# Grid2op/grid2op

Hardware: AMD Instinct MI355X
Metric: env steps/sec (batched DoNothing) (higher is better)
Workload: dtype f64; 1 GPU; l2rpn_case14_sandbox AC Newton-Raphson DoNothing env.step, batch=4096 lanes per GPU; env=l2rpn_case14_sandbox, lanes_per_gpu=4096, total_lanes=4096, env_steps_per_launch=16, observations=every env step -> HBM, cascade=False, kernels=grid-specialised at run time (gpf_jit_enable), parallelism=static lane shards x1, no collective

## Files before the change

grid2op_amd/aot/85d4f0b0125d.h:

```cpp
#define GPF_JIT_SET_G(v) do { (v).n_sub = 118; (v).n_busbar = 2; (v).nb_tot = 236; (v).n_line = 186; (v).n_gen = 62; (v).n_load = 99; (v).n_sto = 7; (v).n_shunt = 14; (v).dim_topo = 540; (v).n_inj = 364; (v).n_out = 2574; (v).n_chron = 322; (v).sn_mva = 0x1p+0; (v).inv_sn_mva = 0x1p+0; } while (0)
#define GPF_JIT_SET_OO(v) do { (v).p_or = 0; (v).q_or = 186; (v).v_or = 372; (v).a_or = 558; (v).th_or = 744; (v).p_ex = 930; (v).q_ex = 1116; (v).v_ex = 1302; (v).a_ex = 1488; (v).th_ex = 1674; (v).gen_p = 1860; (v).gen_q = 1922; (v).gen_v = 1984; (v).gen_th = 2046; (v).load_p = 2108; (v).load_q = 2207; (v).load_v = 2306; (v).load_th = 2405; (v).sto_p = 2504; (v).sto_q = 2511; (v).sto_v = 2518; (v).sto_th = 2525; (v).sh_p = 2532; (v).sh_q = 2546; (v).sh_v = 2560; (v).inj_gen_p = 0; (v).inj_gen_vm = 62; (v).inj_load_p = 124; (v).inj_load_q = 223; (v).inj_sto_p = 322; (v).inj_sto_q = 329; (v).inj_sh_p = 336; (v).inj_sh_q = 350; } while (0)
#define GPF_JIT_SET_SYM(v) do { (v).n = 118; (v).nslot = 674; (v).nslot_y = 476; (v).n_levels = 13; (v).back_off = 2628; (v).n_prog = 3188; (v).scale_off = 2361; (v).n_scale = 267; (v).nslot_lu = 652; (v).n_up = 179; (v).rslot0 = 674; (v).back_first = 11; (v).static_connected = 1; (v).fl[0].n_fwd = 74; (v).fl[0].n_scale = 0; (v).fl[0].n_scale_rhs = 0; (v).fl[0].n_back = 17; (v).fl[0].scale_off = 2400; (v).fl[0].back_off = 2400; (v).fl[0].rhs_field0 = 10784; (v).fl[0].n_words = 3008; (v).fl[0].wave_closed = 1; (v).fl[0].solo_fwd = 0; (v).fl[0].solo_back = 0; (v).fl[1].n_fwd = 39; (v).fl[1].n_scale = 0; (v).fl[1].n_scale_rhs = 0; (v).fl[1].n_back = 11; (v).fl[1].scale_off = 2560; (v).fl[1].back_off = 2560; (v).fl[1].rhs_field0 = 10784; (v).fl[1].n_words = 3392; (v).fl[1].wave_closed = 1; (v).fl[1].solo_fwd = 0; (v).fl[1].solo_back = 0; (v).fl[2].n_fwd = 22; (v).fl[2].n_scale = 0; (v).fl[2].n_scale_rhs = 0; (v).fl[2].n_back = 6; (v).fl[2].scale_off = 2944; (v).fl[2].back_off = 2944; (v).fl[2].rhs_field0 = 10784; (v).fl[2].n_words = 3840; (v).fl[2].wave_closed = 1; (v).fl[2].solo_fwd = 0; (v).fl[2].solo_back = 0; (v).fl[3].n_fwd = 13; (v).fl[3].n_scale = 0; (v).fl[3].n_scale_rhs = 0; (v).fl[3].n_back = 6; (v).fl[3].scale_off = 3584; (v).fl[3].back_off = 3584; (v).fl[3].rhs_field0 = 10784; (v).fl[3].n_words = 5632; (v).fl[3].wave_closed = 1; (v).fl[3].solo_fwd = 7680; (v).fl[3].solo_back = 63; } while (0)
#define GPF_JIT_SET_SO(v) do { (v).n_dbl = 2982; (v).n_int = 6548; (v).n_int_hot = 4024; (v).br_y = 0; (v).br_bdc = 1488; (v).sub_vn_kv = 1674; (v).shunt_fact = 1792; (v).gen_min_q = 1806; (v).gen_max_q = 1868; (v).line_vn = 1930; (v).load_vn = 2674; (v).gen_vn = 2774; (v).sto_vn = 2836; (v).shunt_vn = 2844; (v).line_ka = 2302; (v).gen_qmin_tot = 2858; (v).gen_qmax_tot = 2920; (v).gen_cnt = 5944; (v).dc_inv = -1; (v).line_or_pos = 4024; (v).line_ex_pos = 4212; (v).line_or_sub = 4400; (v).line_ex_sub = 4588; (v).br_slot = 4776; (v).gen_pos = 5520; (v).gen_sub = 5584; (v).gen_slack = 5648; (v).load_pos = 5712; (v).load_sub = 5812; (v).sto_pos = 5912; (v).sto_sub = 5920; (v).shunt_sub = 5928; (v).pair_rc = 3188; (v).up = 3664; (v).prog = 0; (v).pos_line = 6008; } while (0)
```

grid2op_amd/aot/c7e3abcd557d.h:

```cpp
#define GPF_JIT_SET_G(v) do { (v).n_sub = 36; (v).n_busbar = 2; (v).nb_tot = 72; (v).n_line = 59; (v).n_gen = 22; (v).n_load = 37; (v).n_sto = 0; (v).n_shunt = 6; (v).dim_topo = 177; (v).n_inj = 130; (v).n_out = 844; (v).n_chron = 118; (v).sn_mva = 0x1p+0; (v).inv_sn_mva = 0x1p+0; } while (0)
#define GPF_JIT_SET_OO(v) do { (v).p_or = 0; (v).q_or = 59; (v).v_or = 118; (v).a_or = 177; (v).th_or = 236; (v).p_ex = 295; (v).q_ex = 354; (v).v_ex = 413; (v).a_ex = 472; (v).th_ex = 531; (v).gen_p = 590; (v).gen_q = 612; (v).gen_v = 634; (v).gen_th = 656; (v).load_p = 678; (v).load_q = 715; (v).load_v = 752; (v).load_th = 789; (v).sto_p = 826; (v).sto_q = 826; (v).sto_v = 826; (v).sto_th = 826; (v).sh_p = 826; (v).sh_q = 832; (v).sh_v = 838; (v).inj_gen_p = 0; (v).inj_gen_vm = 22; (v).inj_load_p = 44; (v).inj_load_q = 81; (v).inj_sto_p = 118; (v).inj_sto_q = 118; (v).inj_sh_p = 118; (v).inj_sh_q = 124; } while (0)
#define GPF_JIT_SET_SYM(v) do { (v).n = 36; (v).nslot = 196; (v).nslot_y = 146; (v).n_levels = 8; (v).back_off = 752; (v).n_prog = 920; (v).scale_off = 676; (v).n_scale = 76; (v).nslot_lu = 188; (v).n_up = 55; (v).rslot0 = 196; (v).back_first = 6; (v).static_connected = 1; (v).fl[0].n_fwd = 23; (v).fl[0].n_scale = 0; (v).fl[0].n_scale_rhs = 0; (v).fl[0].n_back = 6; (v).fl[0].scale_off = 768; (v).fl[0].back_off = 768; (v).fl[0].rhs_field0 = 3136; (v).fl[0].n_words = 1024; (v).fl[0].wave_closed = 1; (v).fl[0].solo_fwd = 0; (v).fl[0].solo_back = 0; (v).fl[1].n_fwd = 13; (v).fl[1].n_scale = 0; (v).fl[1].n_scale_rhs = 0; (v).fl[1].n_back = 3; (v).fl[1].scale_off = 896; (v).fl[1].back_off = 896; (v).fl[1].rhs_field0 = 3136; (v).fl[1].n_words = 1216; (v).fl[1].wave_closed = 1; (v).fl[1].solo_fwd = 0; (v).fl[1].solo_back = 0; (v).fl[2].n_fwd = 8; (v).fl[2].n_scale = 0; (v).fl[2].n_scale_rhs = 0; (v).fl[2].n_back = 3; (v).fl[2].scale_off = 1152; (v).fl[2].back_off = 1152; (v).fl[2].rhs_field0 = 3136; (v).fl[2].n_words = 1664; (v).fl[2].wave_closed = 1; (v).fl[2].solo_fwd = 0; (v).fl[2].solo_back = 0; (v).fl[3].n_fwd = 8; (v).fl[3].n_scale = 0; (v).fl[3].n_scale_rhs = 0; (v).fl[3].n_back = 3; (v).fl[3].scale_off = 2304; (v).fl[3].back_off = 2304; (v).fl[3].rhs_field0 = 3136; (v).fl[3].n_words = 3584; (v).fl[3].wave_closed = 1; (v).fl[3].solo_fwd = 255; (v).fl[3].solo_back = 7; } while (0)
#define GPF_JIT_SET_SO(v) do { (v).n_dbl = 964; (v).n_int = 2020; (v).n_int_hot = 1180; (v).br_y = 0; (v).br_bdc = 472; (v).sub_vn_kv = 532; (v).shunt_fact = 568; (v).gen_min_q = 574; (v).gen_max_q = 596; (v).line_vn = 618; (v).load_vn = 854; (v).gen_vn = 892; (v).sto_vn = 914; (v).shunt_vn = 914; (v).line_ka = 736; (v).gen_qmin_tot = 920; (v).gen_qmax_tot = 942; (v).gen_cnt = 1816; (v).dc_inv = -2; (v).line_or_pos = 1180; (v).line_ex_pos = 1240; (v).line_or_sub = 1300; (v).line_ex_sub = 1360; (v).br_slot = 1420; (v).gen_pos = 1656; (v).gen_sub = 1680; (v).gen_slack = 1704; (v).load_pos = 1728; (v).load_sub = 1768; (v).sto_pos = 1808; (v).sto_sub = 1808; (v).shunt_sub = 1808; (v).pair_rc = 920; (v).up = 1068; (v).prog = 0; (v).pos_line = 1840; } while (0)
```

grid2op_amd/aot/f41e44a3ff50.h:

```cpp
#define GPF_JIT_SET_G(v) do { (v).n_sub = 118; (v).n_busbar = 2; (v).nb_tot = 236; (v).n_line = 186; (v).n_gen = 62; (v).n_load = 91; (v).n_sto = 7; (v).n_shunt = 14; (v).dim_topo = 532; (v).n_inj = 348; (v).n_out = 2542; (v).n_chron = 306; (v).sn_mva = 0x1p+0; (v).inv_sn_mva = 0x1p+0; } while (0)
#define GPF_JIT_SET_OO(v) do { (v).p_or = 0; (v).q_or = 186; (v).v_or = 372; (v).a_or = 558; (v).th_or = 744; (v).p_ex = 930; (v).q_ex = 1116; (v).v_ex = 1302; (v).a_ex = 1488; (v).th_ex = 1674; (v).gen_p = 1860; (v).gen_q = 1922; (v).gen_v = 1984; (v).gen_th = 2046; (v).load_p = 2108; (v).load_q = 2199; (v).load_v = 2290; (v).load_th = 2381; (v).sto_p = 2472; (v).sto_q = 2479; (v).sto_v = 2486; (v).sto_th = 2493; (v).sh_p = 2500; (v).sh_q = 2514; (v).sh_v = 2528; (v).inj_gen_p = 0; (v).inj_gen_vm = 62; (v).inj_load_p = 124; (v).inj_load_q = 215; (v).inj_sto_p = 306; (v).inj_sto_q = 313; (v).inj_sh_p = 320; (v).inj_sh_q = 334; } while (0)
#define GPF_JIT_SET_SYM(v) do { (v).n = 118; (v).nslot = 674; (v).nslot_y = 476; (v).n_levels = 13; (v).back_off = 2628; (v).n_prog = 3188; (v).scale_off = 2361; (v).n_scale = 267; (v).nslot_lu = 652; (v).n_up = 179; (v).rslot0 = 674; (v).back_first = 11; (v).static_connected = 1; (v).fl[0].n_fwd = 74; (v).fl[0].n_scale = 0; (v).fl[0].n_scale_rhs = 0; (v).fl[0].n_back = 17; (v).fl[0].scale_off = 2400; (v).fl[0].back_off = 2400; (v).fl[0].rhs_field0 = 10784; (v).fl[0].n_words = 3008; (v).fl[0].wave_closed = 1; (v).fl[0].solo_fwd = 0; (v).fl[0].solo_back = 0; (v).fl[1].n_fwd = 39; (v).fl[1].n_scale = 0; (v).fl[1].n_scale_rhs = 0; (v).fl[1].n_back = 11; (v).fl[1].scale_off = 2560; (v).fl[1].back_off = 2560; (v).fl[1].rhs_field0 = 10784; (v).fl[1].n_words = 3392; (v).fl[1].wave_closed = 1; (v).fl[1].solo_fwd = 0; (v).fl[1].solo_back = 0; (v).fl[2].n_fwd = 22; (v).fl[2].n_scale = 0; (v).fl[2].n_scale_rhs = 0; (v).fl[2].n_back = 6; (v).fl[2].scale_off = 2944; (v).fl[2].back_off = 2944; (v).fl[2].rhs_field0 = 10784; (v).fl[2].n_words = 3840; (v).fl[2].wave_closed = 1; (v).fl[2].solo_fwd = 0; (v).fl[2].solo_back = 0; (v).fl[3].n_fwd = 13; (v).fl[3].n_scale = 0; (v).fl[3].n_scale_rhs = 0; (v).fl[3].n_back = 6; (v).fl[3].scale_off = 3584; (v).fl[3].back_off = 3584; (v).fl[3].rhs_field0 = 10784; (v).fl[3].n_words = 5632; (v).fl[3].wave_closed = 1; (v).fl[3].solo_fwd = 7680; (v).fl[3].solo_back = 63; } while (0)
#define GPF_JIT_SET_SO(v) do { (v).n_dbl = 2974; (v).n_int = 6524; (v).n_int_hot = 4024; (v).br_y = 0; (v).br_bdc = 1488; (v).sub_vn_kv = 1674; (v).shunt_fact = 1792; (v).gen_min_q = 1806; (v).gen_max_q = 1868; (v).line_vn = 1930; (v).load_vn = 2674; (v).gen_vn = 2766; (v).sto_vn = 2828; (v).shunt_vn = 2836; (v).line_ka = 2302; (v).gen_qmin_tot = 2850; (v).gen_qmax_tot = 2912; (v).gen_cnt = 5928; (v).dc_inv = -1; (v).line_or_pos = 4024; (v).line_ex_pos = 4212; (v).line_or_sub = 4400; (v).line_ex_sub = 4588; (v).br_slot = 4776; (v).gen_pos = 5520; (v).gen_sub = 5584; (v).gen_slack = 5648; (v).load_pos = 5712; (v).load_sub = 5804; (v).sto_pos = 5896; (v).sto_sub = 5904; (v).shunt_sub = 5912; (v).pair_rc = 3188; (v).up = 3664; (v).prog = 0; (v).pos_line = 5992; } while (0)
```

grid2op_amd/aot/f5e9fdf573e3.h:

```cpp
#define GPF_JIT_SET_G(v) do { (v).n_sub = 14; (v).n_busbar = 2; (v).nb_tot = 28; (v).n_line = 20; (v).n_gen = 6; (v).n_load = 11; (v).n_sto = 0; (v).n_shunt = 1; (v).dim_topo = 57; (v).n_inj = 36; (v).n_out = 271; (v).n_chron = 34; (v).sn_mva = 0x1.9p+6; (v).inv_sn_mva = 0x1.47ae147ae147bp-7; } while (0)
#define GPF_JIT_SET_OO(v) do { (v).p_or = 0; (v).q_or = 20; (v).v_or = 40; (v).a_or = 60; (v).th_or = 80; (v).p_ex = 100; (v).q_ex = 120; (v).v_ex = 140; (v).a_ex = 160; (v).th_ex = 180; (v).gen_p = 200; (v).gen_q = 206; (v).gen_v = 212; (v).gen_th = 218; (v).load_p = 224; (v).load_q = 235; (v).load_v = 246; (v).load_th = 257; (v).sto_p = 268; (v).sto_q = 268; (v).sto_v = 268; (v).sto_th = 268; (v).sh_p = 268; (v).sh_q = 269; (v).sh_v = 270; (v).inj_gen_p = 0; (v).inj_gen_vm = 6; (v).inj_load_p = 12; (v).inj_load_q = 23; (v).inj_sto_p = 34; (v).inj_sto_q = 34; (v).inj_sh_p = 34; (v).inj_sh_q = 35; } while (0)
#define GPF_JIT_SET_SYM(v) do { (v).n = 14; (v).nslot = 66; (v).nslot_y = 54; (v).n_levels = 5; (v).back_off = 242; (v).n_prog = 300; (v).scale_off = 218; (v).n_scale = 24; (v).nslot_lu = 62; (v).n_up = 20; (v).rslot0 = 66; (v).back_first = 3; (v).static_connected = 1; (v).fl[0].n_fwd = 8; (v).fl[0].n_scale = 0; (v).fl[0].n_scale_rhs = 0; (v).fl[0].n_back = 1; (v).fl[0].scale_off = 288; (v).fl[0].back_off = 288; (v).fl[0].rhs_field0 = 1056; (v).fl[0].n_words = 384; (v).fl[0].wave_closed = 1; (v).fl[0].solo_fwd = 0; (v).fl[0].solo_back = 0; (v).fl[1].n_fwd = 5; (v).fl[1].n_scale = 0; (v).fl[1].n_scale_rhs = 0; (v).fl[1].n_back = 1; (v).fl[1].scale_off = 384; (v).fl[1].back_off = 384; (v).fl[1].rhs_field0 = 1056; (v).fl[1].n_words = 576; (v).fl[1].wave_closed = 1; (v).fl[1].solo_fwd = 0; (v).fl[1].solo_back = 0; (v).fl[2].n_fwd = 5; (v).fl[2].n_scale = 0; (v).fl[2].n_scale_rhs = 0; (v).fl[2].n_back = 1; (v).fl[2].scale_off = 768; (v).fl[2].back_off = 768; (v).fl[2].rhs_field0 = 1056; (v).fl[2].n_words = 1024; (v).fl[2].wave_closed = 1; (v).fl[2].solo_fwd = 0; (v).fl[2].solo_back = 0; (v).fl[3].n_fwd = 5; (v).fl[3].n_scale = 0; (v).fl[3].n_scale_rhs = 0; (v).fl[3].n_back = 1; (v).fl[3].scale_off = 1536; (v).fl[3].back_off = 1536; (v).fl[3].rhs_field0 = 1056; (v).fl[3].n_words = 2304; (v).fl[3].wave_closed = 1; (v).fl[3].solo_fwd = 31; (v).fl[3].solo_back = 1; } while (0)
#define GPF_JIT_SET_SO(v) do { (v).n_dbl = 516; (v).n_int = 676; (v).n_int_hot = 396; (v).br_y = 0; (v).br_bdc = 160; (v).sub_vn_kv = 180; (v).shunt_fact = 194; (v).gen_min_q = 196; (v).gen_max_q = 202; (v).line_vn = 208; (v).load_vn = 288; (v).gen_vn = 300; (v).sto_vn = 306; (v).shunt_vn = 306; (v).line_ka = 248; (v).gen_qmin_tot = 308; (v).gen_qmax_tot = 314; (v).gen_cnt = 608; (v).dc_inv = 320; (v).line_or_pos = 396; (v).line_ex_pos = 416; (v).line_or_sub = 436; (v).line_ex_sub = 456; (v).br_slot = 476; (v).gen_pos = 556; (v).gen_sub = 564; (v).gen_slack = 572; (v).load_pos = 580; (v).load_sub = 592; (v).sto_pos = 604; (v).sto_sub = 604; (v).shunt_sub = 604; (v).pair_rc = 300; (v).up = 356; (v).prog = 0; (v).pos_line = 616; } while (0)
```

grid2op_amd/csrc/gridpf_capi.hip:

```cpp
#include <hip/hip_runtime.h>

#include <algorithm>
#include <chrono>
#include <cmath>
#include <cstdio>
#include <cstdlib>
#include <cstring>
#include <climits>
#include <map>
#include <mutex>
#include <string>
#include <vector>

#include "gridpf_engine.hpp"
#include "gridpf_redispatch.hpp"
#include "gridpf_topo.hpp"
#include "gridpf_topo_mask.hpp"

namespace gpf {
__global__ void fanout_kernel(GridDev g, Bufs b, int src, int dst0, int n_dst, const int* __restrict__ out_lines) {
  const int k = blockIdx.x;
  if (k >= n_dst) return;
  const int dst = dst0 + k;
  const int tid = threadIdx.x;
// ... 90 lines not shown
}

namespace {

template <typename T>
hipError_t rows_to_host(const gpf_engine* e, T* host, const DevArr<T>& arr, size_t stride, int lane0, int n) {
  if (!host || stride == 0) return hipSuccess;
  return hipMemcpyAsync(host, arr.p + (size_t)lane0 * stride, (size_t)n * stride * sizeof(T), hipMemcpyDeviceToHost, e->stream);
}
template <typename T>
hipError_t rows_to_device(const gpf_engine* e, const DevArr<T>& arr, const T* host, size_t stride, int lane0, int n) {
  if (!host || stride == 0) return hipSuccess;
  return hipMemcpyAsync(arr.p + (size_t)lane0 * stride, host, (size_t)n * stride * sizeof(T), hipMemcpyHostToDevice, e->stream);
}
template <typename T>
hipError_t rows_copy(const gpf_engine* e, const DevArr<T>& arr, size_t stride, int src, int dst, int n) {
  if (stride == 0) return hipSuccess;
  return hipMemcpyAsync(arr.p + (size_t)dst * stride, arr.p + (size_t)src * stride, (size_t)n * stride * sizeof(T), hipMemcpyDeviceToDevice, e->stream);
}

void topo_unmoved(gpf_engine* e, int lane0, int n) {
  if (e->ta_n_moved == 0) return;
  for (int k = lane0; k < lane0 + n; ++k) if (e->ta_moved[k]) { e->ta_moved[k] = 0; --e->ta_n_moved; }
}

gpf::TopoDev topo_dev(const gpf_engine* e) {
  const gpf::GridDev& g = e->g;
  gpf::TopoDev d{};
  d.dim_topo = g.dim_topo; d.n_line = g.n_line; d.n_sub = g.n_sub; d.n_shunt = g.n_shunt; d.n_busbar = g.n_busbar;
  d.line_or_pos = g.line_or_pos; d.line_ex_pos = g.line_ex_pos; d.shunt_sub = g.shunt_sub;
  d.topo = e->topo.p; d.shunt_bus = e->shunt_bus.p; d.cooldown = e->cooldown.p; d.topo0 = e->topo0.p; d.episode = e->episode.p; d.done = e->done.p;
  return d;
}

gpf::TopoLanes topo_lanes(const gpf_engine* e) {
  gpf::TopoLanes t{};
  t.act = e->ta_act.p; t.sub_cd = e->ta_sub_cd.p; t.last_bus = e->ta_last_bus.p; t.flags = e->ta_flags.p; t.aff = e->ta_aff.p;
  t.ep_snap = e->ta_ep_snap.p; t.list = e->ta_list.p; t.list_rows = e->ta_list_rows.p; t.pos_sub = e->ta_pos_sub.p; t.pos_other = e->ta_pos_other.p;
  t.n_slot = e->ta_n_slot;
  return t;
}

void count_lane(const gpf_engine* e, const int* topo, const int* shunt_bus, int& nb, int& nj, int& mb) {
  const gpf::GridDev& g = e->g;
  std::vector<unsigned char> act(g.nb_tot, 0), type(g.nb_tot, 0);
  auto mark = [&](int sub, int local) -> int {
    if (local < 1 || local > g.n_busbar) return -1;
    int gb = sub + (local - 1) * g.n_sub;
    act[gb] = 1;
    return gb;
  };
  for (int l = 0; l < g.n_line; ++l) {
    int bo = topo[e->h_line_or_pos[l]], be = topo[e->h_line_ex_pos[l]];
    if (bo >= 1 && be >= 1) { mark(e->h_line_or_sub[l], bo); mark(e->h_line_ex_sub[l], be); }
  }
  for (int i = 0; i < g.n_gen; ++i) {
    int gb = mark(e->h_gen_sub[i], topo[e->h_gen_pos[i]]);
    if (gb >= 0) type[gb] = std::max<unsigned char>(type[gb], e->h_gen_slack[i] ? 2 : 1);
  }
  for (int i = 0; i < g.n_load; ++i) mark(e->h_load_sub[i], topo[e->h_load_pos[i]]);
  for (int i = 0; i < g.n_sto; ++i) mark(e->h_sto_sub[i], topo[e->h_sto_pos[i]]);
  if (shunt_bus)
    for (int i = 0; i < g.n_shunt; ++i) mark(e->h_shunt_sub[i], shunt_bus[i]);
  nb = 0;
  nj = 0;
  for (int b = 0; b < g.nb_tot; ++b) {
    if (!act[b]) continue;
    ++nb;
    if (type[b] == 0) nj += 2;
    else if (type[b] == 1) nj += 1;
  }
  mb = 1;
  for (int s = 0; s < g.n_sub; ++s) {
    int c = 0;
    for (int k = 0; k < g.n_busbar; ++k) c += act[s + k * g.n_sub];
    mb = std::max(mb, c);
  }
}



bool upload_flats(const gpf::Symbolic& S, DevArr<int>& buf, gpf::SymDev& D, int lane_opt = 0) {
  D.rslot0 = S.rslot0;
  for (int k = 0; k < 4; ++k) { D.flat[k] = nullptr; D.fl[k] = gpf::FlatDev{}; }
  if (!gpf::flat_fits(S)) return true;
  std::vector<int> all;
  size_t off[4];
  for (int k = 0; k < 4; ++k) {
    static std::mutex cache_mu;
    static std::unordered_map<std::string, gpf::FlatProg> cache;
    std::string key;
    if (lane_opt > 0) {
      key = std::to_string(S.slot_row.size()) + ":" + std::to_string(S.slot_col.size()) + ":" + std::to_string(S.prog.size()) + ":";
      key.append(reinterpret_cast<const char*>(S.slot_row.data()), S.slot_row.size() * sizeof(int));
      key.append(reinterpret_cast<const char*>(S.slot_col.data()), S.slot_col.size() * sizeof(int));
      key.append(reinterpret_cast<const char*>(S.prog.data()), S.prog.size() * sizeof(int));
      key += "/" + std::to_string(16 << k) + "/" + std::to_string(lane_opt) + "/" + std::to_string(S.gj_lv0) + "/" + std::to_string(S.nslot_lu);
    }
    gpf::FlatProg F;
    bool have = false;
    if (lane_opt > 0) {
      std::lock_guard<std::mutex> lk(cache_mu);
      auto hit = cache.find(key);
      if (hit != cache.end()) { F = hit->second; have = true; }
    }
    if (!have) {
      F = gpf::build_flat(S, 16 << k, lane_opt);
      if (lane_opt > 0) {
        std::lock_guard<std::mutex> lk(cache_mu);
        if (cache.size() < 64) cache.emplace(key, F);
      }
    }
    off[k] = all.size();
    all.insert(all.end(), F.words.begin(), F.words.end());
    gpf::FlatDev& f = D.fl[k];
    f.n_fwd = F.n_fwd; f.n_scale = F.n_scale; f.n_scale_rhs = F.n_scale_rhs; f.n_back = F.n_back; f.scale_off = F.scale_off;
    f.back_off = F.back_off; f.rhs_field0 = F.rhs_field0; f.n_words = (int)F.words.size(); f.wave_closed = F.wave_closed ? 1 : 0;
    f.solo_fwd = (int)F.solo_fwd; f.solo_back = (int)F.solo_back;
  }
  if (buf.upload(all.data(), all.size()) != hipSuccess) return false;
  for (int k = 0; k < 4; ++k) D.flat[k] = buf.p + off[k];
  if (g_dry_create) {
    static int dry_words;
    for (int k = 0; k < 4; ++k) D.flat[k] = &dry_words;
  }
  return true;
}

gpf::Symbolic build_symbolic_resident(const gpf::GridDev& g, int n_rows, int n_line, const int* lo, const int* le, bool yb_in_lds);

int topo_class_of(gpf_engine* e, const int* topo, const int* shunt_bus) {
  const gpf::GridDev& g = e->g;
  if (e->no_classes || g.n_busbar < 2 || e->classes.size() >= 8192) return -1;
  const int nbb = g.n_busbar;
  std::string key((size_t)2 * g.n_line + (size_t)g.n_sub * nbb, '\0');
  auto bb = [&](int v) { return v >= 2 && v <= nbb ? v : 1; };
  for (int l = 0; l < g.n_line; ++l) {
    key[2 * l] = (char)bb(topo[e->h_line_or_pos[l]]);
    key[2 * l + 1] = (char)bb(topo[e->h_line_ex_pos[l]]);
  }
  char* used = &key[(size_t)2 * g.n_line];
  auto mark = [&](int sub, int v) { if (v >= 1 && v <= nbb) used[(size_t)sub * nbb + (v - 1)] = 1; };
  for (int l = 0; l < g.n_line; ++l) { mark(e->h_line_or_sub[l], key[2 * l]); mark(e->h_line_ex_sub[l], key[2 * l + 1]); }
  for (int i = 0; i < g.n_gen; ++i) mark(e->h_gen_sub[i], topo[e->h_gen_pos[i]]);
  for (int i = 0; i < g.n_load; ++i) mark(e->h_load_sub[i], topo[e->h_load_pos[i]]);
  for (int i = 0; i < g.n_sto; ++i) mark(e->h_sto_sub[i], topo[e->h_sto_pos[i]]);
  if (shunt_bus) for (int i = 0; i < g.n_shunt; ++i) mark(e->h_shunt_sub[i], shunt_bus[i]);
  std::string elem(used, (size_t)g.n_sub * nbb);
  for (int s_ = 0; s_ < g.n_sub; ++s_) used[(size_t)s_ * nbb] = 1;
  auto it = e->class_of_key.find(key);
  if (it != e->class_of_key.end()) return it->second;
  std::vector<int> node_of((size_t)g.n_sub * nbb, -1);
  int n_nodes = g.n_sub;
  for (int s_ = 0; s_ < g.n_sub; ++s_) node_of[(size_t)s_ * nbb] = s_;
  for (int s_ = 0; s_ < g.n_sub; ++s_)
    for (int k = 1; k < nbb; ++k) if (used[(size_t)s_ * nbb + k]) node_of[(size_t)s_ * nbb + k] = n_nodes++;
  if (n_nodes > 32767) return -1;
  std::vector<int> lo(g.n_line), le(g.n_line);
  for (int l = 0; l < g.n_line; ++l) {
    lo[l] = node_of[(size_t)e->h_line_or_sub[l] * nbb + (key[2 * l] - 1)];
    le[l] = node_of[(size_t)e->h_line_ex_sub[l] * nbb + (key[2 * l + 1] - 1)];
  }
  gpf::Symbolic S = build_symbolic_resident(g, n_nodes, g.n_line, lo.data(), le.data(), true);
  if (S.nslot > 65535 || !gpf::flat_fits(S)) return -1;
  auto c = std::make_unique<gpf_engine::TopoClassHost>();
  std::vector<int> fi;
  auto puti = [&fi](const int* v, size_t n) { int off = (int)fi.size(); fi.insert(fi.end(), v, v + n); while (fi.size() & 3) fi.push_back(0); return off; };
  const int o_prog = puti(S.prog.data(), S.prog.size());
  std::vector<int> rc(S.nslot_y);
  for (int k = 0; k < S.nslot_y; ++k) rc[k] = S.slot_row[k] | (S.slot_col[k] << 16);
  const int o_rc = puti(rc.data(), rc.size());
  const std::vector<int> upv = gpf::build_upairs(S);
  const int o_up = puti(upv.data(), upv.size());
  const int o_br = puti(S.br_slot.data(), S.br_slot.size());
  const int o_no = puti(node_of.data(), node_of.size());
  if (c->tables.upload(fi.data(), fi.size()) != hipSuccess) return -1;
  c->n_nodes = n_nodes; c->nslot = S.nslot; c->nslot_y = S.nslot_y;
  gpf::SymDev& D = c->dev.sym;
  D = e->sym_dev;
  D.n = S.n; D.nslot = S.nslot; D.nslot_lu = S.nslot_lu; D.nslot_y = S.nslot_y; D.n_levels = S.n_levels; D.back_off = S.back_off; D.back_first = S.back_first;
  D.scale_off = S.scale_off; D.n_scale = S.n_scale; D.n_prog = (int)S.prog.size();
  {
    std::vector<int> comp(n_nodes);
    for (int i = 0; i < n_nodes; ++i) comp[i] = i;
    auto find = [&](int x) { while (comp[x] != x) { comp[x] = comp[comp[x]]; x = comp[x]; } return x; };
    for (int l = 0; l < g.n_line; ++l) comp[find(lo[l])] = find(le[l]);
    int root = -1;
    bool one = true;
    for (int s_ = 0; s_ < g.n_sub && one; ++s_)
      for (int k = 0; k < nbb && one; ++k)
        if (elem[(size_t)s_ * nbb + k]) {
          const int r = find(node_of[(size_t)s_ * nbb + k]);
          if (root < 0) root = r; else one = (r == root);
        }
    D.static_connected = one ? 1 : 0;
  }
  D.prog = c->tables.p + o_prog;
  if (!upload_flats(S, c->flat, D) || !D.fl[3].wave_closed) return -1;
  c->dev.pair_rc = c->tables.p + o_rc; c->dev.up = c->tables.p + o_up; c->dev.br_slot = c->tables.p + o_br; c->dev.node_of = c->tables.p + o_no;
  D.n_up = (int)upv.size() / 2;
  const int id = (int)e->classes.size();
// ... 2321 lines not shown
```

grid2op_amd/csrc/gridpf_sparse.hpp:

```cpp
#pragma once
#include <type_traits>
#include "gridpf_common.hpp"

namespace gpf {

struct StatOff {
  int n_dbl, n_int;
  int n_int_hot;
  int br_y, br_bdc, sub_vn_kv, shunt_fact, gen_min_q, gen_max_q;
  int line_vn, load_vn, gen_vn, sto_vn, shunt_vn;
  int line_ka;
  int gen_qmin_tot, gen_qmax_tot;
  int gen_cnt;
  int dc_inv;
  int line_or_pos, line_ex_pos, line_or_sub, line_ex_sub, br_slot, gen_pos, gen_sub, gen_slack, load_pos, load_sub, sto_pos,
      sto_sub, shunt_sub, pair_rc, up, prog;
  int pos_line;
};
#define GPF_STATOFF_INTS(X) X(n_dbl) X(n_int) X(n_int_hot) X(br_y) X(br_bdc) X(sub_vn_kv) X(shunt_fact) X(gen_min_q) X(gen_max_q) X(line_vn) X(load_vn) \
  X(gen_vn) X(sto_vn) X(shunt_vn) X(line_ka) X(gen_qmin_tot) X(gen_qmax_tot) X(gen_cnt) X(dc_inv) X(line_or_pos) X(line_ex_pos) X(line_or_sub) \
  X(line_ex_sub) X(br_slot) X(gen_pos) X(gen_sub) X(gen_slack) X(load_pos) X(load_sub) X(sto_pos) X(sto_sub) X(shunt_sub) X(pair_rc) X(up) X(prog) X(pos_line)
static_assert(sizeof(StatOff) == sizeof(int) * (0 GPF_STATOFF_INTS(GPF_COUNT_FIELD)), "GPF_STATOFF_INTS must list every field of StatOff");
template <class T, bool IN_LDS>
struct SP {
  const T* p;
  __device__ __forceinline__ T operator[](int i) const { return IN_LDS ? p[i] : (T)gptr(p)[i]; }
  __device__ __forceinline__ double4 ld4(size_t off) const {
    if (IN_LDS) return *reinterpret_cast<const double4*>(p + off);
    typedef double v4d_ __attribute__((ext_vector_type(4)));
    const v4d_ v = *(GPF_GLOBAL const v4d_*)(gptr(p) + off);
    return make_double4(v.x, v.y, v.z, v.w);
  }
};
template <int STAGE>
struct StatView {
  static constexpr bool ALL = STAGE == 2, HOT = STAGE >= 1;
  SP<double, ALL> br_y, br_bdc, sub_vn_kv, shunt_fact, gen_min_q, gen_max_q, line_vn, line_ka, load_vn, gen_vn, sto_vn, shunt_vn, dc_inv, gen_qmin_tot, gen_qmax_tot;
  SP<int, ALL> line_or_pos, line_ex_pos, line_or_sub, line_ex_sub, br_slot, gen_pos, gen_sub, gen_slack, load_pos, load_sub,
      sto_pos, sto_sub, shunt_sub, gen_cnt, pos_line;
  SP<int, HOT> pair_rc;
  SP<int, HOT> up;
  SP<int, HOT> prog;
  SP<int, false> node_of;
  SP<double, false> dc_inv_g;
};
template <int STAGE>
__device__ inline void stat_view(StatView<STAGE>& v, const StatOff& o, const double* d, const int* i) {
  v.br_y.p = d + o.br_y; v.br_bdc.p = d + o.br_bdc; v.sub_vn_kv.p = d + o.sub_vn_kv; v.shunt_fact.p = d + o.shunt_fact;
  v.gen_min_q.p = d + o.gen_min_q; v.gen_max_q.p = d + o.gen_max_q;
  v.dc_inv.p = d + (o.dc_inv >= 0 ? o.dc_inv : 0);
  v.gen_qmin_tot.p = d + o.gen_qmin_tot; v.gen_qmax_tot.p = d + o.gen_qmax_tot; v.gen_cnt.p = i + o.gen_cnt;
  v.line_vn.p = d + o.line_vn; v.line_ka.p = d + o.line_ka; v.load_vn.p = d + o.load_vn; v.gen_vn.p = d + o.gen_vn; v.sto_vn.p = d + o.sto_vn; v.shunt_vn.p = d + o.shunt_vn;
  v.line_or_pos.p = i + o.line_or_pos; v.line_ex_pos.p = i + o.line_ex_pos; v.line_or_sub.p = i + o.line_or_sub;
  v.line_ex_sub.p = i + o.line_ex_sub; v.br_slot.p = i + o.br_slot; v.gen_pos.p = i + o.gen_pos; v.gen_sub.p = i + o.gen_sub;
  v.gen_slack.p = i + o.gen_slack; v.load_pos.p = i + o.load_pos; v.load_sub.p = i + o.load_sub; v.sto_pos.p = i + o.sto_pos;
  v.sto_sub.p = i + o.sto_sub; v.shunt_sub.p = i + o.shunt_sub; v.pos_line.p = i + o.pos_line; v.pair_rc.p = i + o.pair_rc; v.up.p = i + o.up; v.prog.p = i + o.prog;
  v.node_of.p = nullptr;
}
__host__ __device__ inline size_t stat_bytes(const StatOff& o, int tier, bool nb1, int n_flat) {
  if (tier == 0) return 0;
  if (!nb1) return ((size_t)o.n_int_hot * 4 + 15) & ~(size_t)15;
  const size_t ints = (size_t)((tier == 2 ? o.n_int : o.n_int_hot) - o.pair_rc) + (size_t)n_flat;
  return ((tier == 2 ? (size_t)o.n_dbl * 8 : 0) + ints * 4 + 15) & ~(size_t)15;
}

struct FlatDev {
  int n_fwd, n_scale, n_scale_rhs, n_back, scale_off, back_off, rhs_field0, n_words;
  int wave_closed;
  int solo_fwd, solo_back;
};
#define GPF_FLATDEV_INTS(X) X(n_fwd) X(n_scale) X(n_scale_rhs) X(n_back) X(scale_off) X(back_off) X(rhs_field0) X(n_words) X(wave_closed) X(solo_fwd) X(solo_back)
static_assert(sizeof(FlatDev) == sizeof(int) * (0 GPF_FLATDEV_INTS(GPF_COUNT_FIELD)), "GPF_FLATDEV_INTS must list every field of FlatDev");
__host__ __device__ constexpr int gw_index(int gw) { return gw >= 128 ? 3 : gw >= 64 ? 2 : gw >= 32 ? 1 : 0; }

struct SymDev {
  int n, nslot, nslot_y, n_levels, back_off, n_prog, scale_off, n_scale;
  int nslot_lu;
  int n_up;
  int rslot0;
  const int* flat[4];
  FlatDev fl[4];
  int back_first;
  int static_connected;
  const int* prog;
  const double* dc_inv_g;
  const double* stat_dbl;
  const int* stat_int;
  StatOff so;
};

#define GPF_SYMDEV_INTS(X) X(n) X(nslot) X(nslot_y) X(n_levels) X(back_off) X(n_prog) X(scale_off) X(n_scale) X(nslot_lu) X(n_up) X(rslot0) X(back_first) \
  X(static_connected)

struct TopoClassDev {
  SymDev sym;
  const int* pair_rc;
  const int* up;
  const int* br_slot;
  const int* node_of;
};

struct DevParamsS {
  GridDev g;
  Bufs b;
  OutOff oo;
  SymDev sym;
  const TopoClassDev* classes;
  int tc_rows;
  int tc_nslot, tc_nslot_y;
  int dcf;
  EnvDyn env;
};

#ifdef GPF_TIMING
constexpr int GPF_NSTAMP = 40;
constexpr int GPF_NPASS_T = 48;
constexpr int GPF_WORK_ROW = GPF_NSTAMP + GPF_NPASS_T;
static __shared__ long long gpf_pass_t[GPF_NPASS_T];
struct Stamps { long long v[GPF_NSTAMP]; };
#define GPF_STAMPS(k) do { stamps.v[(k)] = (long long)__builtin_readcyclecounter(); } while (0)
#define GPF_STAMPS_PARAM , Stamps& stamps
#define GPF_STAMPS_ARG , stamps
#define GPF_STAMPS_DECL Stamps stamps; for (int k_ = 0; k_ < GPF_NSTAMP; ++k_) stamps.v[k_] = 0; \
  for (int k_ = threadIdx.x; k_ < GPF_NPASS_T; k_ += blockDim.x) gpf_pass_t[k_] = 0
#define GPF_STAMPS_FLUSH(inst_) do { if (tid == 0) { for (int k_ = 0; k_ < GPF_NSTAMP; ++k_) P->b.work[(size_t)(inst_) * GPF_WORK_ROW + k_] = (double)stamps.v[k_]; \
    for (int k_ = 0; k_ < GPF_NPASS_T; ++k_) P->b.work[(size_t)(inst_) * GPF_WORK_ROW + GPF_NSTAMP + k_] = (double)gpf_pass_t[k_]; } } while (0)
#else
#define GPF_STAMPS(k) do {} while (0)
#define GPF_STAMPS_PARAM
#define GPF_STAMPS_ARG
#define GPF_STAMPS_DECL do {} while (0)
#define GPF_STAMPS_FLUSH(inst_) do {} while (0)
#endif

#ifndef GPF_WAVE_SYNC
#define GPF_SYNC() __syncthreads()
#else
#define GPF_SYNC() do { __builtin_amdgcn_fence(__ATOMIC_RELEASE, "wavefront"); __builtin_amdgcn_wave_barrier(); \
                        __builtin_amdgcn_fence(__ATOMIC_ACQUIRE, "wavefront"); } while (0)
#endif

#ifndef GPF_HARD_SYNC
#define GPF_PF2_ON true
#define GPF_LSYNC() do { if (GW > WAVE) asm volatile("s_waitcnt lgkmcnt(0)\n\ts_barrier" ::: "memory"); else { asm volatile("" ::: "memory"); __builtin_amdgcn_wave_barrier(); asm volatile("" ::: "memory"); } } while (0)
#else
#define GPF_PF2_ON false
#define GPF_LSYNC() GPF_SYNC()
#endif

#define GPF_SYNC_IF(cond) do { if (GW > WAVE || (cond)) GPF_SYNC(); else GPF_LSYNC(); } while (0)

typedef short i16;

#ifndef GPF_JIT
__device__ __forceinline__ void pin_sgpr(int& x) { x = __builtin_amdgcn_readfirstlane(x); asm volatile("" : "+s"(x)); }
#define GPF_SPEC_G(v) do {} while (0)
#define GPF_SPEC_OO(v) do {} while (0)
#define GPF_SPEC_SYM(v) do {} while (0)
#define GPF_SPEC_SO(v) do {} while (0)
#else
__device__ __forceinline__ void pin_sgpr(int&) {}
#define GPF_SPEC_G(v) GPF_JIT_SET_G(v)
#define GPF_SPEC_OO(v) GPF_JIT_SET_OO(v)
#define GPF_SPEC_SYM(v) GPF_JIT_SET_SYM(v)
#define GPF_SPEC_SO(v) GPF_JIT_SET_SO(v)
#endif

template <int NB>
struct CarveP {
  static constexpr int BS = 2 * NB;
  double* A;
  double* Yb;
  double* rhs;
  double *vm, *va, *e, *f, *Psp, *Qsp;
  double* ivm;
  double *Sre, *Sim;
  double* Gs;
  double* inj;
  double* Adc;
  int* btype;
  int* vidx;
  int* lab;
  int* topo;
  i16 *lor_b, *lex_b, *gen_b, *load_b, *sto_b, *sh_b;
  i8* sub_bb;
  float* out_l;
};

template <int NB>
__host__ __device__ inline size_t lds_bytes_instance(const GridDev& g, int nslot, int nslot_y, bool stage_inj, int n_rows = -1, bool dcf = false) {
  constexpr int BS = 2 * NB;
  const size_t rows = n_rows > 0 ? (size_t)n_rows : (size_t)g.n_sub;
  const size_t nbus = rows * NB;
  const size_t rs0 = (size_t)nslot > (3 * rows + 1) / 2 ? (size_t)nslot : (3 * rows + 1) / 2;
  size_t a_d = NB == 1 ? (rs0 + rows) * 4 : (size_t)nslot * BS * BS;
  const size_t topo_d = (((size_t)g.dim_topo + 1) / 2 + 2) & ~(size_t)1;
  if (a_d < topo_d) a_d = topo_d;
  const size_t nd = a_d + (size_t)nslot_y * NB * NB * 2 + (NB == 1 ? 7 * nbus : rows * BS + 8 * nbus) + (stage_inj ? (size_t)g.n_inj : 0) +
// ... 333 lines not shown
#pragma unroll
        for (int m = 0; m < BS; ++m) acc = fma(Di[m], bp[m], acc);
      }
      GPF_LSYNC();
      if (on) rhs[(size_t)p * BS + (it % BS)] = acc;
      GPF_LSYNC();
    }
    }
    for (int it = tid; it < n_c * B2; it += GW) {
      const int o = it / B2, r = (it % B2) / BS, q = it % BS;
      const unsigned w0 = (unsigned)prog[c_off + 2 * o];
      const int u = prog[c_off + 2 * o + 1] & 0xffff;
      const double* Al = A + (size_t)(w0 >> 16) * B2 + r * BS;
      const double* Au = A + (size_t)u * B2 + q;
      double acc = 0.0;
#pragma unroll
      for (int m = 0; m < BS; ++m) acc = fma(Al[m], Au[m * BS], acc);
      atomicAdd(&A[(size_t)(w0 & 0xffffu) * B2 + r * BS + q], -acc);
    }
    for (int it = tid; it < n_r * BS; it += GW) {
      const int o = it / BS, r = it % BS;
      const unsigned w0 = (unsigned)prog[r_off + 2 * o];
      const int p = prog[r_off + 2 * o + 1];
      const double* Al = A + (size_t)(w0 & 0xffffu) * B2 + r * BS;
      const double* bp = rhs + (size_t)p * BS;
      double acc = 0.0;
#pragma unroll
      for (int m = 0; m < BS; ++m) acc = fma(Al[m], bp[m], acc);
      atomicAdd(&rhs[(size_t)(w0 >> 16) * BS + r], -acc);
    }
    GPF_LSYNC();
  }
#ifdef GPF_TIMING
  const long long t_lu1 = __builtin_readcyclecounter();
#endif
  for (int lv = S.n_levels - 1; lv >= 0; --lv) {
    const int ent_off = prog[S.back_off + 2 * lv], n_ent = prog[S.back_off + 2 * lv + 1];
    for (int it = tid; it < n_ent * BS; it += GW) {
      const unsigned w = (unsigned)prog[ent_off + 2 * (it / BS)];
      const int p = prog[ent_off + 2 * (it / BS) + 1], r = it % BS;
      const double* Au = A + (size_t)(w & 0xffffu) * B2 + r * BS;
      const double* xj = rhs + (size_t)(w >> 16) * BS;
      double acc = 0.0;
#pragma unroll
      for (int m = 0; m < BS; ++m) acc = fma(Au[m], xj[m], acc);
      atomicAdd(&rhs[(size_t)p * BS + r], -acc);
    }
    GPF_LSYNC();
  }
#ifdef GPF_TIMING
  if (dbg) { dbg[0] = t_lu1 - t_lu0; dbg[1] = (long long)__builtin_readcyclecounter() - t_lu1; }
#endif
  return ok;
}

constexpr int GPF_WR_CAP_F = 6, GPF_WR_CAP_B = 2;
template <bool ON> struct FlatWords { };
template <> struct FlatWords<true> { unsigned f[2 * GPF_WR_CAP_F], b[2 * GPF_WR_CAP_B]; };
#ifdef GPF_NO_WORDS_RES
template <int NB, int IPW, int WPI> constexpr bool flat_words_ct() { return false; }
#else
template <int NB, int IPW, int WPI> constexpr bool flat_words_ct() { return NB == 1 && IPW > 1 && WPI == 1; }
#endif
__device__ __forceinline__ bool flat_words_fit(const FlatDev& F) { return F.n_fwd <= GPF_WR_CAP_F && F.n_back <= GPF_WR_CAP_B; }
template <int GW, class PP>
__device__ __forceinline__ void flat_words_load(FlatWords<false>&, const FlatDev&, PP, int) {}
template <int GW, class PP>
__device__ __forceinline__ void flat_words_load(FlatWords<true>& W, const FlatDev& F, PP prog, int tid) {
  const bool fit = flat_words_fit(F);
#pragma unroll
  for (int k = 0; k < GPF_WR_CAP_F; ++k) {
    const bool on_f = fit && k < F.n_fwd;
    W.f[2 * k] = on_f ? (unsigned)prog[2 * tid + 2 * GW * k] : 0xffffffffu;
    W.f[2 * k + 1] = on_f ? (unsigned)prog[2 * tid + 2 * GW * k + 1] : 0u;
  }
#pragma unroll
  for (int k = 0; k < GPF_WR_CAP_B; ++k) {
    const bool on_b = fit && k < F.n_back;
    W.b[2 * k] = on_b ? (unsigned)prog[F.back_off + 2 * tid + 2 * GW * k] : 0xffffffffu;
    W.b[2 * k + 1] = on_b ? (unsigned)prog[F.back_off + 2 * tid + 2 * GW * k + 1] : 0u;
  }
}

template <int GW, class PP = const int*, bool RES = false>
__device__ inline bool block_lu_flat(const FlatDev& F, PP prog, double* __restrict__ A, size_t HS, int tid, long long* dbg = nullptr,
                                     const FlatWords<RES>* W = nullptr) {
#ifdef GPF_TIMING
  const long long t_lu0 = __builtin_readcyclecounter();
#endif
  bool ok = true;
#ifdef GPF_PF2_IG
  constexpr bool PF2 = GPF_PF2_ON && (GW > WAVE || (GW <= 32 && !std::is_same<PP, const int*>::value));
#else
  constexpr bool PF2 = GPF_PF2_ON && GW > WAVE;
#endif
  char* const a0 = reinterpret_cast<char*>(A);
  char* const a1 = a0 + HS * 8;
#define FL_LD2(base, f) (*reinterpret_cast<const double2*>((base) + (f)))
#define FL_D(base, f) (reinterpret_cast<double*>((base) + (f)))
#ifdef GPF_TIMING
#define GPF_PASS_T(i_) do { if (dbg && tid == 0 && (i_) < GPF_NPASS_T) gpf_pass_t[(i_)] = (long long)__builtin_readcyclecounter(); } while (0)
#else
#define GPF_PASS_T(i_) do {} while (0)
#endif
  GPF_PASS_T(0);
  auto fwd_item = [&](const unsigned w0, const unsigned w1) {
    if (w0 != 0xffffffffu) {
      const unsigned fd = w0 & 0xffffu, fl = w0 >> 16, fu = w1 & 0xffffu, fp = w1 >> 16;
      const double2 dA = FL_LD2(a0, fp), dB = FL_LD2(a1, fp), lA = FL_LD2(a0, fl), lB = FL_LD2(a1, fl);
      const double2 uA = FL_LD2(a0, fu), uB = FL_LD2(a1, fu);
      const double rd = -fast_rcp(fma(dA.x, dB.y, -dA.y * dB.x));
      const double t00 = fma(lA.x, dB.y, -lA.y * dB.x), t01 = fma(lA.y, dA.x, -lA.x * dA.y);
      const double t10 = fma(lB.x, dB.y, -lB.y * dB.x), t11 = fma(lB.y, dA.x, -lB.x * dA.y);
      double* d0_ = FL_D(a0, fd);
      double* d1_ = FL_D(a1, fd);
      atomicAdd(&d0_[0], fma(t00, uA.x, t01 * uB.x) * rd);
      atomicAdd(&d1_[0], fma(t10, uA.x, t11 * uB.x) * rd);
      if (fd < (unsigned)F.rhs_field0) {
        atomicAdd(&d0_[1], fma(t00, uA.y, t01 * uB.y) * rd);
        atomicAdd(&d1_[1], fma(t10, uA.y, t11 * uB.y) * rd);
      }
    }
  };
#define GPF_WALK(n_, at0_, MASK_, NEXT_SOLO_, ITEM_, TB_, WR_, CAP_)                                                                                 \
  {                                                                                                                                \
    const unsigned solo_ = GW > WAVE ? (unsigned)(MASK_) : 0u;                                                                     \
    const int n_pass_ = (n_);                                                                                                      \
    auto step_ = [&](const unsigned a_, const unsigned b_, const int k) {                                                          \
      const bool so_ = GW > WAVE && k < 32 && ((solo_ >> (k & 31)) & 1u);                                                          \
      if (!so_ || tid < WAVE) ITEM_(a_, b_);                                                                                       \
      const bool sn_ = so_ && (k + 1 < n_pass_ ? (k + 1 < 32 && ((solo_ >> ((k + 1) & 31)) & 1u)) : (GW > WAVE && (NEXT_SOLO_)));  \
      if (sn_) { asm volatile("" ::: "memory"); __builtin_amdgcn_wave_barrier(); asm volatile("" ::: "memory"); }                 \
      else GPF_LSYNC();                                                                                                            \
      GPF_PASS_T((TB_) + k);                                                                                                       \
    };                                                                                                                             \
    if constexpr (RES) {                                   \
      _Pragma("unroll")                                                                                                            \
      for (int k = 0; k < (CAP_); ++k)                                                                                             \
        if (k < n_pass_) step_(W->WR_[2 * k], W->WR_[2 * k + 1], k);                                                               \
    } else {                                                                                                                       \
    int at = (at0_) + 2 * tid;                                                                                                     \
    unsigned p0 = (unsigned)prog[at], p1 = (unsigned)prog[at + 1];                                                                 \
    if (PF2) {                                                                                                                     \
      at += 2 * GW;                                                                                                                \
      unsigned q0 = (unsigned)prog[at], q1 = (unsigned)prog[at + 1], r0, r1;                                                       \
      for (int k = 0; k < n_pass_; k += 3) {                                                                                       \
        at += 2 * GW; r0 = (unsigned)prog[at]; r1 = (unsigned)prog[at + 1];                                                        \
        step_(p0, p1, k);                                                                                                          \
        if (k + 1 >= n_pass_) break;                                                                                               \
        at += 2 * GW; p0 = (unsigned)prog[at]; p1 = (unsigned)prog[at + 1];                                                        \
        step_(q0, q1, k + 1);                                                                                                      \
        if (k + 2 >= n_pass_) break;                                                                                               \
        at += 2 * GW; q0 = (unsigned)prog[at]; q1 = (unsigned)prog[at + 1];                                                        \
        step_(r0, r1, k + 2);                                                                                                      \
      }                                                                                                                            \
    } else {                                                                                                                       \
      for (int k = 0; k < n_pass_; ++k) {                                                                                          \
        at += 2 * GW;                                                                                                              \
        const unsigned n0 = (unsigned)prog[at], n1 = (unsigned)prog[at + 1];                           \
        step_(p0, p1, k);                                                                                                          \
        p0 = n0; p1 = n1;                                                                                                          \
      }                                                                                                                            \
    }                                                                                                                              \
    }                                                                                                                              \
  }
  GPF_WALK(F.n_fwd, 0, F.solo_fwd, F.n_back > 0 && (F.solo_back & 1), fwd_item, 1, f, GPF_WR_CAP_F)
#ifdef GPF_TIMING
  const long long t_lu1 = __builtin_readcyclecounter();
#endif
  auto back_item = [&](const unsigned w0, const unsigned w1) {
    if (w0 != 0xffffffffu) {
      const unsigned fu = w0 & 0xffffu, fj = w0 >> 16, fdj = fj - (unsigned)F.rhs_field0;
      const double2 uA = FL_LD2(a0, fu), uB = FL_LD2(a1, fu), dA = FL_LD2(a0, fdj), dB = FL_LD2(a1, fdj);
      const double s0 = *FL_D(a0, fj), s1 = *FL_D(a1, fj);
      const double rd = fast_rcp(fma(dA.x, dB.y, -dA.y * dB.x));
      const double x0 = fma(dB.y, s0, -dA.y * s1) * rd, x1 = fma(dA.x, s1, -dB.x * s0) * rd;
      atomicAdd(FL_D(a0, w1), -fma(uA.x, x0, uA.y * x1));
      atomicAdd(FL_D(a1, w1), -fma(uB.x, x0, uB.y * x1));
    }
  };
  GPF_WALK(F.n_back, F.back_off, F.solo_back, false, back_item, 1 + F.n_fwd, b, GPF_WR_CAP_B)
#ifdef GPF_TIMING
  if (dbg) { dbg[0] = t_lu1 - t_lu0; dbg[1] = (long long)__builtin_readcyclecounter() - t_lu1; }
#endif
  return ok;
}

template <int GW, bool FACTOR, bool COMPACT, class PP = const int*, bool RES = false>
__device__ inline bool scalar_lu_flat(const FlatDev& F, PP prog, double* __restrict__ A, double* __restrict__ fac, int tid,
                                      long long* dbg = nullptr, const FlatWords<RES>* W = nullptr) {
#ifdef GPF_TIMING
  const long long t_lu0 = __builtin_readcyclecounter();
#endif
  bool ok = true;
#ifdef GPF_PF2_IG
  constexpr bool PF2 = GPF_PF2_ON && (GW > WAVE || (GW <= 32 && !std::is_same<PP, const int*>::value));
#else
  constexpr bool PF2 = GPF_PF2_ON && GW > WAVE;
#endif
  char* const a0 = reinterpret_cast<char*>(A);
  char* const fb = reinterpret_cast<char*>(fac);
  auto facp = [&](unsigned f) -> double* { return reinterpret_cast<double*>(fb + (COMPACT ? (f >> 1) : f)); };
  auto fwd_item = [&](const unsigned w0, const unsigned w1) {
    const unsigned fd = w0 & 0xffffu, fl = w0 >> 16, fu = w1 & 0xffffu, fp = w1 >> 16;
    const bool is_r = (int)fd >= F.rhs_field0;
    if (w0 != 0xffffffffu && (FACTOR || is_r)) {
      const double d = *facp(fp), al = *facp(fl);
      const double x = is_r ? *FL_D(a0, fu) : *facp(fu);
      double* dst = is_r ? FL_D(a0, fd) : facp(fd);
      atomicAdd(dst, -(al * x) * fast_rcp(d));
    }
  };
#undef GPF_PASS_T
#define GPF_PASS_T(i_) do {} while (0)
  GPF_WALK(F.n_fwd, 0, F.solo_fwd, F.n_back > 0 && (F.solo_back & 1), fwd_item, 0, f, GPF_WR_CAP_F)
#ifdef GPF_TIMING
  const long long t_lu1 = __builtin_readcyclecounter();
#endif
  auto back_item = [&](const unsigned w0, const unsigned w1) {
    if (w0 != 0xffffffffu) {
      const unsigned fj = w0 >> 16;
      atomicAdd(FL_D(a0, w1), -(*facp(w0 & 0xffffu) * *FL_D(a0, fj)) * fast_rcp(*facp(fj - (unsigned)F.rhs_field0)));
    }
  };
  GPF_WALK(F.n_back, F.back_off, F.solo_back, false, back_item, 0, b, GPF_WR_CAP_B)
#ifdef GPF_TIMING
  if (dbg) { dbg[0] = t_lu1 - t_lu0; dbg[1] = (long long)__builtin_readcyclecounter() - t_lu1; }
#endif
  return ok;
}
#undef GPF_PASS_T
#undef GPF_WALK
#undef FL_LD2
#undef FL_D

struct SolveCtl {
  bool inj_staged;
  bool topo_staged;
  bool reuse;
  bool dcf;
  bool write_bus;
  bool sums_done;
  bool warm;
  bool otraj;
  int orow;
  bool write_topo;
  bool inj_regs;
  float r_lp0, r_lq0, r_lp1, r_lq1, r_pp, r_vm;
  bool tc_rebuild;
};
struct TopoState {
  int status;
  int nb;
  bool dc_base;
  int dc_out;
  bool gen_base;
  int tc[2];
};

constexpr int YR_PASSES = 4;
template <int NB, int STAGE, int IPW, int WPI, bool TC, bool YR = false>
__device__ inline int solve_instance_sparse(const DevParamsS* __restrict__ P, const SymDev& S, const FlatDev& FL, const StatView<STAGE>& sv, CarveP<NB>& c, double2* yreg, unsigned* rcreg,
                                            const FlatWords<flat_words_ct<NB, IPW, WPI>()>& FW, int inst, int is_dc, int max_iter,
                                            double tol_pu, int tid, const SolveCtl& ctl, TopoState& ts, int& n_iter_out, int& nb_out, float& a_or_first GPF_STAMPS_PARAM) {
  typedef Grp<IPW, WPI> G;
  constexpr int GW = G::GW;
  constexpr int BS = 2 * NB;
  constexpr int B2 = BS * BS;
  GridDev g_loc = P->g;
  GPF_SPEC_G(g_loc);
  pin_sgpr(g_loc.n_sub); pin_sgpr(g_loc.n_line); pin_sgpr(g_loc.n_gen); pin_sgpr(g_loc.n_load); pin_sgpr(g_loc.n_sto);
  pin_sgpr(g_loc.n_shunt); pin_sgpr(g_loc.dim_topo); pin_sgpr(g_loc.nb_tot);
  const GridDev& g = g_loc;
  const Bufs& b = P->b;
#ifdef GPF_JIT
  OutOff oo_loc = P->oo;
  GPF_SPEC_OO(oo_loc);
  const OutOff& oo = oo_loc;
#else
  const OutOff& oo = P->oo;
#endif
  const int nsub = g.n_sub;
  const int nbus = TC ? S.n : nsub * NB;
  constexpr int GWA = WPI > 1 ? WAVE : GW;
  const bool acc_lane = WPI == 1 || tid < WAVE;
  const bool wave1 = WPI > 1 && tid >= WAVE;
  const size_t HS = ((size_t)S.rslot0 + S.n) * 2;
  auto bel = [&](int slot, int r, int col) -> double* {
    return BS == 2 ? c.A + (size_t)r * HS + (size_t)slot * 2 + col : c.A + (size_t)slot * B2 + r * BS + col;
  };
  auto rhsT = [&](int i) -> double* { return BS == 2 ? c.A + ((size_t)S.rslot0 + i) * 2 : c.rhs + (size_t)(i / NB) * BS + 2 * (i % NB); };
  auto rhsV = [&](int i) -> double* { return BS == 2 ? c.A + HS + ((size_t)S.rslot0 + i) * 2 : c.rhs + (size_t)(i / NB) * BS + 2 * (i % NB) + 1; };
  auto SreP = [&](int i) -> double* { return BS == 2 ? c.A + ((size_t)S.rslot0 + i) * 2 + 1 : c.Sre + i; };
  auto SimP = [&](int i) -> double* { return BS == 2 ? c.A + HS + ((size_t)S.rslot0 + i) * 2 + 1 : c.Sim + i; };
  auto EF = [&](int i) -> double2 { return NB == 1 ? reinterpret_cast<const double2*>(c.e)[i] : make_double2(c.e[i], c.f[i]); };
  auto setEF = [&](int i, double e_, double f_) { if (NB == 1) reinterpret_cast<double2*>(c.e)[i] = make_double2(e_, f_); else { c.e[i] = e_; c.f[i] = f_; } };
  const auto topo_g = gptr(b.topo) + (size_t)inst * g.dim_topo;
  const auto shb = gptr(b.shunt_bus) + (size_t)inst * g.n_shunt;
  n_iter_out = 0;
  nb_out = 0;
  c.out_l = nullptr;
  GPF_STAMPS(0);
  const auto inj_g = gptr(b.inj) + (size_t)inst * g.n_inj;
  if (STAGE && !ctl.inj_staged) {
    for (int i = tid; i < g.n_inj; i += GW) c.inj[i] = inj_g[i];
  }
  const bool reuse = ctl.reuse;
  const bool dc_kept = reuse && ctl.dcf && NB == 1;
  const bool warm = reuse && ctl.warm && !is_dc;
#ifdef GPF_NO_NWR
  constexpr bool NWR = false;
#else
  constexpr bool NWR = NB == 1 && WPI == 1 && !YR;
#endif
  const bool nwr = NWR && !is_dc && nbus <= GW && S.n_up <= GW;
  const bool fast_pre = nwr && reuse && ctl.sums_done && !warm && !TC && S.so.dc_inv != -1 && G::block_all_u(ts.dc_base && ts.dc_out < 0);
#define GPF_INJ(i_) (STAGE ? c.inj[(i_)] : (double)inj_g[(i_)])
// ... 194 lines not shown
  if (!dc_skip) for (int i = tid; i < (NB == 1 ? S.nslot : S.nslot_lu) * B2; i += GW) c.A[i] = 0.0;
  if (do_y) for (int i = tid; i < S.nslot_y * NB * NB * 2; i += GW) ydst[i] = 0.0;
  GPF_LSYNC();
  if (acc_lane)
  for (int l = tid; l < g.n_line; l += GWA) {
    const int f = c.lor_b[l], t = c.lex_b[l];
    if (f < 0) continue;
    const int bi = lidx(f), bj = lidx(t);
    const int sff = sv.br_slot[4 * l + 0], sft = sv.br_slot[4 * l + 1], stf = sv.br_slot[4 * l + 2], stt = sv.br_slot[4 * l + 3];
    if (do_y) {
      const double4 ya = sv.br_y.ld4((size_t)8 * l), yb = sv.br_y.ld4((size_t)8 * l + 4);
      double* y;
      y = ydst + ((size_t)sff * NB * NB + bi * NB + bi) * 2; atomicAdd(&y[0], ya.x); atomicAdd(&y[1], ya.y);
      y = ydst + ((size_t)sft * NB * NB + bi * NB + bj) * 2; atomicAdd(&y[0], ya.z); atomicAdd(&y[1], ya.w);
      y = ydst + ((size_t)stf * NB * NB + bj * NB + bi) * 2; atomicAdd(&y[0], yb.x); atomicAdd(&y[1], yb.y);
      y = ydst + ((size_t)stt * NB * NB + bj * NB + bj) * 2; atomicAdd(&y[0], yb.z); atomicAdd(&y[1], yb.w);
    }
    if (f != t && !dc_skip) {
      const double bb = sv.br_bdc[l];
      const bool ff_ = c.btype[f] != BT_REF, tf_ = c.btype[t] != BT_REF;
      const int rf = 2 * bi, rt = 2 * bj;
      if (ff_) atomicAdd(bel(sff, rf, rf), bb);
      if (tf_) atomicAdd(bel(stt, rt, rt), bb);
      if (ff_ && tf_) {
        atomicAdd(bel(sft, rf, rt), -bb);
        atomicAdd(bel(stf, rt, rf), -bb);
      }
    }
  }
  if (do_y && acc_lane) {
    for (int s = tid; s < g.n_shunt; s += GWA) {
      const int bu = c.sh_b[s];
      if (bu >= 0) {
        const int bi = lidx(bu);
        const int sub = (NB == 1) ? bu : bu / NB;
        const double fct = sv.shunt_fact[s] * inv_sn;
        double* y = ydst + ((size_t)sub * NB * NB + bi * NB + bi) * 2;
        atomicAdd(&y[0], GPF_INJ(oo.inj_sh_p + s) * fct);
        atomicAdd(&y[1], -GPF_INJ(oo.inj_sh_q + s) * fct);
      }
    }
  }
  GPF_LSYNC();
  if (YR && do_y) {
#pragma unroll
    for (int k = 0; k < YR_PASSES; ++k) {
      const int pr = tid + k * GW;
      const unsigned w0 = pr < S.n_up ? (unsigned)sv.up[2 * pr] : 0u, w1 = pr < S.n_up ? (unsigned)sv.up[2 * pr + 1] : 0u;
      rcreg[2 * k] = w0; rcreg[2 * k + 1] = w1;
      yreg[2 * k] = pr < S.n_up ? *reinterpret_cast<const double2*>(ydst + (size_t)(w1 & 0xffffu) * 2) : make_double2(0.0, 0.0);
      yreg[2 * k + 1] = pr < S.n_up ? *reinterpret_cast<const double2*>(ydst + (size_t)(w1 >> 16) * 2) : make_double2(0.0, 0.0);
    }
    yreg[2 * YR_PASSES] = tid < nbus ? *reinterpret_cast<const double2*>(ydst + (size_t)tid * 2) : make_double2(0.0, 0.0);
    GPF_LSYNC();
  }
  }
  if (!fuse_dc)
  for (int i = tid; i < nbus; i += GW) {
    const int sub = (NB == 1) ? i : i / NB, bi = lidx(i);
    const int bt = c.btype[i];
    const bool th_live = (bt == BT_PQ || bt == BT_PV);
    if (!dc_skip) {
      if (!th_live) *bel(sub, 2 * bi, 2 * bi) = 1.0;
      *bel(sub, 2 * bi + 1, 2 * bi + 1) = 1.0;
    }
    *rhsT(i) = th_live ? (c.Psp[i] - c.Gs[i]) : 0.0;
    *rhsV(i) = 0.0;
  }
  if (!fuse_dc) GPF_LSYNC();
  }
  GPF_STAMPS(3);
  const int* const flat_g = STAGE == 0 ? sv.prog.p : S.flat[gw_index(GW)];
  constexpr bool PROG_LDS = STAGE >= 1 && IPW == 1;
  constexpr bool WRES = flat_words_ct<NB, IPW, WPI>();
  const bool wres = WRES && flat_words_fit(FL);
  auto lu_ac = [&](long long* dbg) -> bool {
    if (BS == 2) {
      if (WRES && wres) return block_lu_flat<GW, decltype(gptr(flat_g)), WRES>(FL, gptr(flat_g), c.A, HS, tid, dbg, &FW);
      if (PROG_LDS) return block_lu_flat<GW>(FL, sv.prog.p, c.A, HS, tid, dbg);
      return block_lu_flat<GW>(FL, gptr(flat_g), c.A, HS, tid, dbg);
    }
    if (STAGE >= 1) return block_lu_solve<BS, GW>(S, sv.prog.p, c.A, c.rhs, tid, dbg);
    return block_lu_solve<BS, GW>(S, gptr(sv.prog.p), c.A, c.rhs, tid, dbg);
  };
  auto lu_dc = [&](long long* dbg) -> bool {
    if (dc_kept) {
      if (WRES && wres) return scalar_lu_flat<GW, false, true, decltype(gptr(flat_g)), WRES>(FL, gptr(flat_g), c.A, c.Adc, tid, dbg, &FW);
      if (PROG_LDS) return scalar_lu_flat<GW, false, true>(FL, sv.prog.p, c.A, c.Adc, tid, dbg);
      return scalar_lu_flat<GW, false, true>(FL, gptr(flat_g), c.A, c.Adc, tid, dbg);
    }
    if (WRES && wres) return scalar_lu_flat<GW, true, false, decltype(gptr(flat_g)), WRES>(FL, gptr(flat_g), c.A, c.A, tid, dbg, &FW);
    if (PROG_LDS) return scalar_lu_flat<GW, true, false>(FL, sv.prog.p, c.A, c.A, tid, dbg);
    return scalar_lu_flat<GW, true, false>(FL, gptr(flat_g), c.A, c.A, tid, dbg);
  };
  if (!warm && !fuse_dc) {
#ifdef GPF_TIMING
    bool ok = dc_inv ? true : (NB == 1) ? lu_dc(&stamps.v[20])
                                        : lu_ac(&stamps.v[20]);
#else
    bool ok = dc_inv ? true : (NB == 1) ? lu_dc(nullptr) : lu_ac(nullptr);
#endif
    for (int i = tid; i < nbus; i += GW) {
      double th;
      if (dc_inv) {
        auto row_times_rhs = [&](const auto tab) -> double {
          double t0 = 0.0, t1 = 0.0;
          for (int k0 = 0; k0 < nbus; k0 += MVC) {
            double a_[MVC], r_[MVC];
#pragma unroll
            for (int q = 0; q < MVC; ++q) {
              const int k = k0 + q < nbus ? k0 + q : nbus - 1;
              a_[q] = tab[k * nbus + i];
              r_[q] = *rhsT(k);
            }
#pragma unroll
            for (int q = 0; q < MVC; q += 2) {
              if (k0 + q < nbus) t0 = fma(a_[q], r_[q], t0);
              if (k0 + q + 1 < nbus) t1 = fma(a_[q + 1], r_[q + 1], t1);
            }
          }
          return t0 + t1;
        };
        th = S.so.dc_inv >= 0 ? row_times_rhs(sv.dc_inv) : row_times_rhs(sv.dc_inv_g);
      } else if (NB == 1) {
        const double d = dc_kept ? c.Adc[i] : c.A[(size_t)i * 2];
        if (!(fabs(d) > 1e-300) || !(fabs(d) < 1e300)) ok = false;
        th = *rhsT(i) * fast_rcp(d);
      } else th = *rhsT(i);
      const int bt = c.btype[i];
      c.va[i] = (bt == BT_PQ || bt == BT_PV) ? th : 0.0;
      if (bt != BT_OFF && !(fabs(th) < 1e300)) ok = false;
    }
    if (NB == 1 && ctl.dcf && !dc_skip)
      for (int q = tid; q < S.nslot; q += GW) c.Adc[q] = c.A[(size_t)q * 2];
    GPF_LSYNC();
    if (WPI == 1 && dc_inv && G::block_any_u(ts.dc_out >= 0)) {
      const int lo_ = ts.dc_out >= 0 ? ts.dc_out : 0;
      const int f_ = sv.line_or_sub[lo_], t_ = sv.line_ex_sub[lo_];
      const double bl = ts.dc_out >= 0 ? sv.br_bdc[lo_] : 0.0;
      const bool f_ref = c.btype[f_] == BT_REF, t_ref = c.btype[t_] == BT_REF;
      const double dth = c.va[f_] - c.va[t_];
      const double xff = f_ref ? 0.0 : dcinv(f_ * nbus + f_), xtt = t_ref ? 0.0 : dcinv(t_ * nbus + t_);
      const double xft = (f_ref || t_ref) ? 0.0 : dcinv(t_ * nbus + f_);
      const double den = 1.0 - bl * (xff - 2.0 * xft + xtt);
      if (!(fabs(den) > 1e-12)) ok = false;
      const double kk = bl * dth / den;
      for (int i = tid; i < nbus; i += GW) {
        const int bt = c.btype[i];
        const double u_ = (f_ref ? 0.0 : dcinv(f_ * nbus + i)) - (t_ref ? 0.0 : dcinv(t_ * nbus + i));
        if (bt == BT_PQ || bt == BT_PV) c.va[i] += u_ * kk;
      }
      GPF_LSYNC();
    }
    if (status == 0 && G::any(!ok)) status = 4;
    if (G::block_all_u(status != 0)) return status;
  }
  GPF_STAMPS(4);

  int it = 0;
  if (!is_dc) {
    bool converged = false;
    bool done = status != 0;
    const int n_pairs = S.nslot_y * NB * NB;
    auto t_of = [&](const double2 y, double ei, double fi, double ej, double fj, double& tr_, double& ti_) {
      const double aa = y.x * ej - y.y * fj, bb = y.x * fj + y.y * ej;
      tr_ = ei * aa + fi * bb;
      ti_ = fi * aa - ei * bb;
    };
    if (nwr) {
      const bool p_on = tid < S.n_up, b_on = tid < nbus;
      const int ib = b_on ? tid : 0;
      const unsigned w0 = p_on ? (unsigned)sv.up[2 * tid] : 0u, w1 = p_on ? (unsigned)sv.up[2 * tid + 1] : 0u;
      const int u = (int)(w0 & 0xffffu), v = (int)(w0 >> 16), suv = (int)(w1 & 0xffffu), svu = (int)(w1 >> 16);
      constexpr bool KEEP_Y = IPW > 1;
      const double2* const p_yuv = reinterpret_cast<const double2*>(c.Yb + (size_t)suv * 2);
      const double2* const p_yvu = reinterpret_cast<const double2*>(c.Yb + (size_t)svu * 2);
      const double2* const p_yd = reinterpret_cast<const double2*>(c.Yb + (size_t)ib * 2);
      const double2 yuv0 = *p_yuv, yvu0 = *p_yvu, ydiag0 = *p_yd;
      const int btu = c.btype[u], btv = c.btype[v];
      const int bt = c.btype[ib];
      const double psp0 = c.Psp[ib], qsp0 = c.Qsp[ib];
#define NWR_YUV (KEEP_Y ? yuv0 : *p_yuv)
#define NWR_YVU (KEEP_Y ? yvu0 : *p_yvu)
#define NWR_YD (KEEP_Y ? ydiag0 : *p_yd)
#define NWR_PSP (KEEP_Y ? psp0 : c.Psp[ib])
#define NWR_QSP (KEEP_Y ? qsp0 : c.Qsp[ib])
      double va, vm;
#ifdef GPF_TIMING
      asm volatile("s_waitcnt lgkmcnt(0)" ::: "memory");
      GPF_STAMPS(20);
#endif
      if (fuse_dc) {
        const int vi = fast_pre ? c.vidx[ib] : -1;
        const double vm_lds = fast_pre ? 1.0 : c.vm[ib];
        if (b_on) c.ivm[ib] = psp0 - c.Gs[ib];
        GPF_LSYNC();
        auto row_times_rhs = [&](const auto tab, const bool by_row) -> double {
          double t0 = 0.0, t1 = 0.0;
          for (int k0 = 0; k0 < nbus; k0 += MVC) {
            double a_[MVC], r_[MVC];
#pragma unroll
            for (int q = 0; q < MVC; ++q) {
              const int k = k0 + q < nbus ? k0 + q : nbus - 1;
              a_[q] = by_row ? tab[ib * nbus + k] : tab[k * nbus + ib];
              r_[q] = c.ivm[k];
            }
#pragma unroll
            for (int q = 0; q < MVC; q += 2) {
              if (k0 + q < nbus) t0 = fma(a_[q], r_[q], t0);
              if (k0 + q + 1 < nbus) t1 = fma(a_[q + 1], r_[q + 1], t1);
            }
          }
          return t0 + t1;
        };
        const double th = S.so.dc_inv >= 0 ? row_times_rhs(sv.dc_inv, STAGE == 2) : row_times_rhs(sv.dc_inv_g, false);
        const bool live = (bt == BT_PQ || bt == BT_PV);
        va = live ? th : 0.0;
        vm = (vi >= 0 && (bt == BT_PV || bt == BT_REF)) ? GPF_INJ(oo.inj_gen_vm + vi) : vm_lds;
        const bool th_bad = b_on && bt != BT_OFF && !(fabs(th) < 1e300);
        if (status == 0 && G::any(th_bad)) { status = 4; done = true; }
      } else { va = c.va[ib]; vm = c.vm[ib]; }
#ifdef GPF_TIMING
      GPF_STAMPS(21);
#endif
      const bool act = p_on && (btu != BT_OFF) && (btv != BT_OFF);
      const bool uP = (btu == BT_PQ || btu == BT_PV), uQ = (btu == BT_PQ), vP = (btv == BT_PQ || btv == BT_PV), vQ = (btv == BT_PQ);
      const bool acc_u = act && (yuv0.x != 0.0 || yuv0.y != 0.0), acc_v = act && (yvu0.x != 0.0 || yvu0.y != 0.0);
      const bool rowP = (bt == BT_PQ || bt == BT_PV), rowQ = (bt == BT_PQ);
      const bool diag_on = bt != BT_OFF && (ydiag0.x != 0.0 || ydiag0.y != 0.0);
      double* const Ad0 = bel(ib, 0, 0);
      double* const Ad1 = bel(ib, 1, 0);
      double* const b_uv0 = bel(suv, 0, 0); double* const b_uv1 = bel(suv, 1, 0);
      double* const b_vu0 = bel(svu, 0, 0); double* const b_vu1 = bel(svu, 1, 0);
      double e, f, ivm, Sr = 0.0, Si = 0.0;
      {
        double sn_, co;
        fast_sincos(va, sn_, co);
        e = vm * co; f = vm * sn_; ivm = fast_rcp(vm);
        if (b_on) { setEF(ib, e, f); c.ivm[ib] = ivm; *SreP(ib) = 0.0; *SimP(ib) = 0.0; }
      }
      for (int i = S.nslot_y * 2 + tid; i < S.nslot * 2; i += GW) { c.A[i] = 0.0; c.A[HS + i] = 0.0; }
      GPF_LSYNC();
      GPF_STAMPS(10);
      asm volatile("; GPF_NEWTON_NWR_BEGIN" ::: "memory");
      while (true) {
        if (p_on) {
          const double2 efu = EF(u), efv = EF(v);
          const double ivmu = c.ivm[u], ivmv = c.ivm[v];
          double tr_, ti_, sr_, si_;
          const double2 yuv = NWR_YUV, yvu = NWR_YVU;
          t_of(yuv, efu.x, efu.y, efv.x, efv.y, tr_, ti_);
          t_of(yvu, efv.x, efv.y, efu.x, efu.y, sr_, si_);
          *reinterpret_cast<double2*>(b_uv0) = make_double2((uP && vP) ? ti_ : 0.0, (uP && vQ) ? tr_ * ivmv : 0.0);
          *reinterpret_cast<double2*>(b_uv1) = make_double2((uQ && vP) ? -tr_ : 0.0, (uQ && vQ) ? ti_ * ivmv : 0.0);
          *reinterpret_cast<double2*>(b_vu0) = make_double2((vP && uP) ? si_ : 0.0, (vP && uQ) ? sr_ * ivmu : 0.0);
          *reinterpret_cast<double2*>(b_vu1) = make_double2((vQ && uP) ? -sr_ : 0.0, (vQ && uQ) ? si_ * ivmu : 0.0);
          if (acc_u) { atomicAdd(SreP(u), tr_); atomicAdd(SimP(u), ti_); }
          if (acc_v) { atomicAdd(SreP(v), sr_); atomicAdd(SimP(v), si_); }
        }
        GPF_LSYNC();
        if (it == 0) GPF_STAMPS(11);
        double fabs_mis = 0.0;
        bool bad = false;
        if (b_on) {
          Sr = *SreP(ib); Si = *SimP(ib);
          const double2 ydiag = NWR_YD;
          const double psp = NWR_PSP, qsp = NWR_QSP;
          double tr_, ti_;
          t_of(ydiag, e, f, e, f, tr_, ti_);
          if (diag_on) { Sr += tr_; Si += ti_; }
          const double2 r0 = make_double2(rowP ? ti_ : 0.0, (rowP && rowQ) ? tr_ * ivm : 0.0);
          const double2 r1 = make_double2((rowQ && rowP) ? -tr_ : 0.0, rowQ ? ti_ * ivm : 0.0);
          *reinterpret_cast<double2*>(Ad0) = make_double2(rowP ? r0.x - Si : 1.0, rowQ ? fma(Sr, ivm, r0.y) : r0.y);
          *reinterpret_cast<double2*>(Ad1) = make_double2(rowQ ? r1.x + Sr : r1.x, rowQ ? fma(Si, ivm, r1.y) : 1.0);
          const double mp = rowP ? (Sr - psp) : 0.0;
          const double mq = rowQ ? (Si - qsp) : 0.0;
          *rhsT(ib) = -mp; *rhsV(ib) = -mq;
          const double am = fmax(fabs(mp), fabs(mq));
          if (!(am <= 1e300)) bad = true;
          fabs_mis = am;
        }
        if (!done) {
          const unsigned fl = G::template any2<0>(!(fabs_mis < tol_pu), bad);
          if (fl & 2u) { status = 1; done = true; }
          else if (!(fl & 1u)) { converged = true; done = true; }
          else if (it >= max_iter) done = true;
          else ++it;
        }
        if (G::block_all_u(done)) break;
        GPF_LSYNC();
        if (it == 1) GPF_STAMPS(12);
#ifdef GPF_TIMING
        const bool ok = lu_ac(it == 1 ? &stamps.v[32] : nullptr);
#else
        const bool ok = lu_ac(nullptr);
#endif
        if (it == 1) GPF_STAMPS(13);
        bool fin = true, piv_ok = true;
        if (b_on) {
          double2 dx = make_double2(*rhsT(ib), *rhsV(ib));
          const double2 dA = *reinterpret_cast<const double2*>(Ad0), dB = *reinterpret_cast<const double2*>(Ad1);
          const double det = fma(dA.x, dB.y, -dA.y * dB.x);
          if (!(fabs(det) > 1e-300) || !(fabs(det) < 1e300)) piv_ok = false;
          const double rd = fast_rcp(det);
          dx = make_double2(fma(dB.y, dx.x, -dA.y * dx.y) * rd, fma(dA.x, dx.y, -dB.x * dx.x) * rd);
          if (!done && bt != BT_OFF) {
            if (!(fabs(dx.x) < 1e300) || !(fabs(dx.y) < 1e300)) fin = false;
            if (bt == BT_PQ || bt == BT_PV) va += dx.x;
            if (bt == BT_PQ) vm += dx.y;
            if (vm < 0.0) { vm = -vm; va += 3.14159265358979323846; }
            if (fabs(va) > 3.14159265358979323846) va = remainder(va, 6.28318530717958647692);
          }
          double sn_, co;
          fast_sincos(va, sn_, co);
          e = vm * co; f = vm * sn_; ivm = fast_rcp(vm);
          setEF(ib, e, f);
          c.ivm[ib] = ivm;
          *SreP(ib) = 0.0;
          *SimP(ib) = 0.0;
        }
        for (int i = S.nslot_y * 2 + tid; i < S.nslot * 2; i += GW) { c.A[i] = 0.0; c.A[HS + i] = 0.0; }
        GPF_LSYNC();
        if (!done && G::template any2<1>(!ok || !piv_ok, !fin) != 0u) { status = 4; done = true; }
        if (it == 1) GPF_STAMPS(14);
        asm volatile("; GPF_NEWTON_NWR_BACKEDGE" ::: "memory");
      }
      if (b_on) { *SreP(ib) = Sr; *SimP(ib) = Si; c.va[ib] = va; c.vm[ib] = vm; }
#undef NWR_YUV
#undef NWR_YVU
#undef NWR_YD
#undef NWR_PSP
#undef NWR_QSP
    } else {
      for (int i = tid; i < nbus; i += GW) {
        const double va = c.va[i], vmi = c.vm[i];
        double sn_, co;
        fast_sincos(va, sn_, co);
        setEF(i, vmi * co, vmi * sn_);
        if (NB == 1) c.ivm[i] = fast_rcp(vmi);
        *SreP(i) = 0.0;
        *SimP(i) = 0.0;
        if (WPI > 1) { *rhsT(i) = 0.0; *rhsV(i) = 0.0; }
      }
      if (BS == 2) { for (int i = S.nslot_y * 2 + tid; i < S.nslot * 2; i += GW) { c.A[i] = 0.0; c.A[HS + i] = 0.0; } }
      else for (int i = S.nslot_y * B2 + tid; i < S.nslot_lu * B2; i += GW) c.A[i] = 0.0;
      GPF_LSYNC();
      GPF_STAMPS(10);
      unsigned rc_first = 0, rc_first1 = 0;
      if (STAGE == 0 && !YR) {
        if (NB == 1) { if (tid < S.n_up) { rc_first = (unsigned)sv.up[2 * tid]; rc_first1 = (unsigned)sv.up[2 * tid + 1]; } }
        else if (tid < n_pairs) rc_first = (unsigned)sv.pair_rc[tid / (NB * NB)];
      }
      while (true) {
        if (NB == 1) {
          auto upair_item = [&](const unsigned w0, const unsigned w1, const double2 yuv, const double2 yvu) {
            const int u = (int)(w0 & 0xffffu), v = (int)(w0 >> 16), suv = (int)(w1 & 0xffffu), svu = (int)(w1 >> 16);
            const int btu = c.btype[u], btv = c.btype[v];
            const double2 efu = EF(u), efv = EF(v);
            const double eu = efu.x, fu = efu.y, ivmu = c.ivm[u], ev = efv.x, fv = efv.y, ivmv = c.ivm[v];
            double tr_, ti_, sr_, si_;
            t_of(yuv, eu, fu, ev, fv, tr_, ti_);
            t_of(yvu, ev, fv, eu, fu, sr_, si_);
            const bool act = (btu != BT_OFF) && (btv != BT_OFF);
            const bool uP = (btu == BT_PQ || btu == BT_PV), uQ = (btu == BT_PQ), vP = (btv == BT_PQ || btv == BT_PV), vQ = (btv == BT_PQ);
            *reinterpret_cast<double2*>(bel(suv, 0, 0)) = make_double2((uP && vP) ? ti_ : 0.0, (uP && vQ) ? tr_ * ivmv : 0.0);
            *reinterpret_cast<double2*>(bel(suv, 1, 0)) = make_double2((uQ && vP) ? -tr_ : 0.0, (uQ && vQ) ? ti_ * ivmv : 0.0);
            *reinterpret_cast<double2*>(bel(svu, 0, 0)) = make_double2((vP && uP) ? si_ : 0.0, (vP && uQ) ? sr_ * ivmu : 0.0);
            *reinterpret_cast<double2*>(bel(svu, 1, 0)) = make_double2((vQ && uP) ? -sr_ : 0.0, (vQ && uQ) ? si_ * ivmu : 0.0);
            if (act && (yuv.x != 0.0 || yuv.y != 0.0)) { atomicAdd(wave1 ? rhsT(u) : SreP(u), tr_); atomicAdd(wave1 ? rhsV(u) : SimP(u), ti_); }
            if (act && (yvu.x != 0.0 || yvu.y != 0.0)) { atomicAdd(wave1 ? rhsT(v) : SreP(v), sr_); atomicAdd(wave1 ? rhsV(v) : SimP(v), si_); }
          };
          if (YR && S.n_up <= 2 * GW) {
            struct PairOps { int btu, btv; double2 efu, efv; double ivmu, ivmv; };
            auto pair_load = [&](const unsigned w0) -> PairOps {
              const int u = (int)(w0 & 0xffffu), v = (int)(w0 >> 16);
              PairOps o;
              o.btu = c.btype[u]; o.btv = c.btype[v]; o.efu = EF(u); o.efv = EF(v); o.ivmu = c.ivm[u]; o.ivmv = c.ivm[v];
              return o;
            };
            auto pair_fin = [&](const PairOps& o, const unsigned w0, const unsigned w1, const double2 yuv, const double2 yvu) {
              const int u = (int)(w0 & 0xffffu), v = (int)(w0 >> 16), suv = (int)(w1 & 0xffffu), svu = (int)(w1 >> 16);
              const int btu = o.btu, btv = o.btv;
              const double eu = o.efu.x, fu = o.efu.y, ivmu = o.ivmu, ev = o.efv.x, fv = o.efv.y, ivmv = o.ivmv;
              double tr_, ti_, sr_, si_;
              t_of(yuv, eu, fu, ev, fv, tr_, ti_);
              t_of(yvu, ev, fv, eu, fu, sr_, si_);
              const bool act = (btu != BT_OFF) && (btv != BT_OFF);
              const bool uP = (btu == BT_PQ || btu == BT_PV), uQ = (btu == BT_PQ), vP = (btv == BT_PQ || btv == BT_PV), vQ = (btv == BT_PQ);
              *reinterpret_cast<double2*>(bel(suv, 0, 0)) = make_double2((uP && vP) ? ti_ : 0.0, (uP && vQ) ? tr_ * ivmv : 0.0);
              *reinterpret_cast<double2*>(bel(suv, 1, 0)) = make_double2((uQ && vP) ? -tr_ : 0.0, (uQ && vQ) ? ti_ * ivmv : 0.0);
              *reinterpret_cast<double2*>(bel(svu, 0, 0)) = make_double2((vP && uP) ? si_ : 0.0, (vP && uQ) ? sr_ * ivmu : 0.0);
              *reinterpret_cast<double2*>(bel(svu, 1, 0)) = make_double2((vQ && uP) ? -sr_ : 0.0, (vQ && uQ) ? si_ * ivmu : 0.0);
              if (act && (yuv.x != 0.0 || yuv.y != 0.0)) { atomicAdd(wave1 ? rhsT(u) : SreP(u), tr_); atomicAdd(wave1 ? rhsV(u) : SimP(u), ti_); }
              if (act && (yvu.x != 0.0 || yvu.y != 0.0)) { atomicAdd(wave1 ? rhsT(v) : SreP(v), sr_); atomicAdd(wave1 ? rhsV(v) : SimP(v), si_); }
            };
            const bool on0 = tid < S.n_up, on1 = tid + GW < S.n_up;
            const PairOps o0 = pair_load(rcreg[0]), o1 = pair_load(rcreg[2]);
            if (on0) pair_fin(o0, rcreg[0], rcreg[1], yreg[0], yreg[1]);
            if (on1) pair_fin(o1, rcreg[2], rcreg[3], yreg[2], yreg[3]);
          } else if (YR) {
  #pragma unroll
            for (int k = 0; k < YR_PASSES; ++k) if (tid + k * GW < S.n_up) upair_item(rcreg[2 * k], rcreg[2 * k + 1], yreg[2 * k], yreg[2 * k + 1]);
          } else {
            unsigned p0 = rc_first, p1 = rc_first1;
            for (int k = tid; k < S.n_up; k += GW) {
              unsigned w0, w1;
              if (STAGE == 0) { w0 = p0; w1 = p1; if (k + GW < S.n_up) { p0 = (unsigned)sv.up[2 * (k + GW)]; p1 = (unsigned)sv.up[2 * (k + GW) + 1]; } }
              else { w0 = (unsigned)sv.up[2 * k]; w1 = (unsigned)sv.up[2 * k + 1]; }
              upair_item(w0, w1, *reinterpret_cast<const double2*>(c.Yb + (size_t)(w1 & 0xffffu) * 2),
                         *reinterpret_cast<const double2*>(c.Yb + (size_t)(w1 >> 16) * 2));
            }
          }
        } else {
          auto pair_item = [&](int pr, const double2 y, const unsigned rc) {
            const int slot = pr / (NB * NB), bi = (pr / NB) % NB, bj = pr % NB;
// ... 840 lines not shown
  bool env_fail = false;
  constexpr bool PF9 = WPI == 1;
  float pf_lp = 0.f, pf_lq = 0.f, pf_pp = 0.f, pf_pv = 1.f;
  if (PF9) {
    const auto ch0 = gptr(b.chron) + ((size_t)tab * sa.T + row) * g.n_chron;
    if (tid < g.n_load) { pf_lp = ch0[tid]; pf_lq = ch0[g.n_load + tid]; }
    if (tid < g.n_gen) { pf_pp = ch0[2 * g.n_load + tid]; pf_pv = ch0[2 * g.n_load + g.n_gen + tid]; }
  }
  bool keep_hit = false, keep_dirty = false;
  bool keep_claim = false;
  GPF_STAMPS(34);
  if (keep_on) {
    const auto kb = (GPF_GLOBAL const unsigned char*)sa.keep.p + (YR ? (size_t)sa.keep.stride : 0);
    const auto kt = (GPF_GLOBAL const int*)kb + KEEP_HDR_INTS;
    bool same = k_same;
#pragma unroll
    for (int u = 0; u < KT; ++u) same &= kk[u] == tn[u];
    {
      const auto topo_now = gptr(b.topo) + (size_t)inst * g.dim_topo;
      const auto shb_now = gptr(b.shunt_bus) + (size_t)inst * g.n_shunt;
      const auto kd = (GPF_GLOBAL const double*)(kb + sa.keep.off_kd);
      const auto inj_now = gptr(b.inj) + (size_t)inst * g.n_inj + oo.inj_sh_p;
      for (int i = tid + KT * GW; i < g.dim_topo; i += GW) same &= kt[i] == topo_now[i];
      for (int i = tid + GW; i < g.n_shunt; i += GW) same &= kt[g.dim_topo + i] == shb_now[i];
      for (int i = tid + 2 * GW; i < 2 * g.n_shunt; i += GW) same &= kd[i] == inj_now[i];
    }
    GPF_STAMPS(36);
    const bool valid = k_h0 > KEEP_VALID && k_h0 - KEEP_VALID < sa.keep.launch;
    {
      const auto km16 = (GPF_GLOBAL const v4i_*)(kb + sa.keep.off_m);
      const auto ky = (GPF_GLOBAL const v2d_*)(kb + sa.keep.off_y);
      const auto ka = (GPF_GLOBAL const double*)(kb + sa.keep.off_d);
      int* const img = c.btype;
      v2i_* const img2 = reinterpret_cast<v2i_*>(img);
      const int n_m = sa.keep.n_m;
      auto put4 = [&](int ch, const v4i_ t_) {
        if (4 * ch + 3 < n_m) { img2[2 * ch] = v2i_{t_.x, t_.y}; img2[2 * ch + 1] = v2i_{t_.z, t_.w}; }
        else { if (4 * ch < n_m) img[4 * ch] = t_.x; if (4 * ch + 1 < n_m) img[4 * ch + 1] = t_.y; if (4 * ch + 2 < n_m) img[4 * ch + 2] = t_.z; }
      };
      const int n_ch = (n_m + 3) >> 2;
#pragma unroll
      for (int u = 0; u < KC; ++u) { const int ch = tid + u * GW; if (ch < n_ch) put4(ch, im[u]); }
      for (int ch = tid + KC * GW; ch < n_ch; ch += GW) put4(ch, km16[ch]);
      if (!YR) {
        double2* const yl = reinterpret_cast<double2*>(c.Yb);
#pragma unroll
        for (int u = 0; u < KY; ++u) { const int i = tid + u * GW; if (i < S.nslot_y) yl[i] = yy[u]; }
        for (int i = tid + KY * GW; i < S.nslot_y; i += GW) { const v2d_ t_ = ky[i]; yl[i] = make_double2(t_.x, t_.y); }
      }
      if (keep_dcf && (k_h2 & 4)) {
#pragma unroll
        for (int u = 0; u < KA; ++u) { const int q = tid + u * GW; if (q < S.nslot) c.Adc[q] = aa[u]; }
        for (int q = tid + KA * GW; q < S.nslot; q += GW) c.Adc[q] = ka[q];
      }
    }
    GPF_STAMPS(37);
    const unsigned hb = G::template any_bits<3, 4>(((same && valid) ? 0u : 1u) | ((k_h2 & 1) ? 0u : 2u) | ((k_h2 & 4) ? 0u : 4u) | (same ? 0u : 8u));
    const unsigned hbb = IPW == 1 ? hb : ((__any(hb & 1u) ? 1u : 0u) | (__any(hb & 2u) ? 2u : 0u) | (__any(hb & 4u) ? 4u : 0u));
    keep_hit = !(hbb & 1u) && (!keep_dcf || !(hbb & 2u) || !(hbb & 4u));
    keep_claim = !(hb & 8u) && k_h0 == KEEP_KEYED && !ghost;
    if (keep_hit) {
      ts.status = k_h1 & 0xff; ts.nb = k_h1 >> 8; ts.dc_base = (k_h2 & 1) != 0; ts.gen_base = (k_h2 & 2) != 0; ts.dc_out = (k_h2 >> 3) - 1;
      reuse = true;
    }
    GPF_STAMPS(38);
    GPF_LSYNC();
  }
  GPF_STAMPS(39);
#define GPF_REDERIVE()                                                                                              \
  do {                                                                                                              \
    grp = grp0; tid = tid0; inst = inst0;                                                                           \
    asm volatile("" : "+v"(grp), "+v"(tid), "+v"(inst));                                                            \
    carve_sparse<NB>(c, smem + (size_t)grp * per_inst, g, lds_nslot, lds_nslot_y, STAGE != 0, lds_rows, lds_dcf);   \
  } while (0)
  const bool tobs = b.traj_out != nullptr;
  FlatWords<flat_words_ct<NB, IPW, WPI>()> FW;
  flat_words_load<GW>(FW, FL, gptr(S.flat[GWI]), tid0);
  for (int step = 0; step < sa.n_steps; ++step) {
    GPF_REDERIVE();
    const bool last = step + 1 == sa.n_steps;
    const bool otraj = tobs && step < b.traj_cap;
    int orow = otraj ? step * (int)b.lane_stride + inst : inst;
    GPF_STAMPS(19);
    bool sums_in_k9 = false, skip_inj = false;
    float k9_lp0 = 0.f, k9_lq0 = 0.f, k9_lp1 = 0.f, k9_lq1 = 0.f, k9_pp = 0.f, k9_vm = 1.f;
    {
      const auto ch = gptr(b.chron) + ((size_t)tab * sa.T + row) * g.n_chron;
      const auto sc = gptr(b.lane_scale) + (size_t)inst * 2 * g.n_load;
      const auto gdelta = gptr(b.lane_gen_delta) + (size_t)inst * g.n_gen;
      const auto inj_g = gptr(b.inj) + (size_t)inst * g.n_inj;
      bool any_maint = false;
      const auto mrow = gptr(b.maint) + ((size_t)tab * sa.T + row) * g.n_line;
      if (b.maint) {
        const auto topo = gptr(b.topo) + (size_t)inst * g.dim_topo;
        bool hit = false;
        if (!ghost)
        for (int l = tid; l < g.n_line; l += GW)
          if (mrow[l] && topo[sv.line_or_pos[l]] != -1) { topo[sv.line_or_pos[l]] = -1; topo[sv.line_ex_pos[l]] = -1; hit = true; }
        any_maint = G::block_any(hit);
        if (any_maint) reuse = false;
      }
      if (!reuse) { const auto topo = gptr(b.topo) + (size_t)inst * g.dim_topo; for (int i = tid; i < g.dim_topo; i += GW) c.topo[i] = topo[i]; }
      if (any_maint) {
        GPF_SYNC();
        for (int l = tid; l < g.n_line; l += GW) if (mrow[l]) { c.topo[sv.line_or_pos[l]] = -1; c.topo[sv.line_ex_pos[l]] = -1; }
      }
      float pp_pre = pf_pp, pv_pre = pf_pv, lp_pre = pf_lp, lq_pre = pf_lq;
      constexpr bool PRE2 = WPI > 1;
      constexpr int gw9 = WPI > 1 ? WAVE : GW;
      float lp2 = 0.f, lq2 = 0.f, sc2p = 1.f, sc2q = 1.f;
      if (!PF9) {
        pp_pre = tid < g.n_gen ? ch[2 * g.n_load + tid] : 0.f;
        pv_pre = tid < g.n_gen ? ch[2 * g.n_load + g.n_gen + tid] : 1.f;
        if (PRE2 && tid < gw9) {
          if (tid < g.n_load) { lp_pre = ch[tid]; lq_pre = ch[g.n_load + tid]; }
          if (tid + gw9 < g.n_load) {
            lp2 = ch[tid + gw9]; lq2 = ch[g.n_load + tid + gw9];
            if (has_sc) { sc2p = sc[tid + gw9]; sc2q = sc[g.n_load + tid + gw9]; }
          }
        }
      }
      if (PF9 && !last) {
        const int row_n = row + 1 >= sa.T ? 0 : row + 1;
        const auto chn = gptr(b.chron) + ((size_t)tab * sa.T + row_n) * g.n_chron;
        if (tid < g.n_load) { pf_lp = chn[tid]; pf_lq = chn[g.n_load + tid]; }
        if (tid < g.n_gen) { pf_pp = chn[2 * g.n_load + tid]; pf_pv = chn[2 * g.n_load + g.n_gen + tid]; }
      }
      double sum_load = 0.0, sum_prod = 0.0;
      sums_in_k9 = reuse;
      skip_inj = WPI > 1 && !STAGE && sums_in_k9 && !last && !env_on && sa.cascade == 0 && g.n_load <= 2 * WAVE && g.n_gen <= WAVE;
      const double inv_sn9 = g.inv_sn_mva;
      if (sums_in_k9) {
        const int nbus9 = TC ? S.n : g.n_sub * NB;
        for (int i = tid; i < nbus9; i += GW) { c.Psp[i] = 0.0; c.Qsp[i] = 0.0; c.Gs[i] = 0.0; }
        GPF_LSYNC();
      }
      GPF_STAMPS(16);
      const bool lane9 = tid < gw9;
      if (lane9)
      for (int i = tid; i < g.n_load; i += gw9) {
        const bool i0_ = (PF9 || PRE2) && i == tid, i1_ = PRE2 && i == tid + gw9;
        float lp = i0_ ? lp_pre : i1_ ? lp2 : ch[i], lq = i0_ ? lq_pre : i1_ ? lq2 : ch[g.n_load + i];
        if (has_sc) { lp *= (i == tid) ? sc_p0 : i1_ ? sc2p : sc[i]; lq *= (i == tid) ? sc_q0 : i1_ ? sc2q : sc[g.n_load + i]; }
        if (STAGE) { c.inj[oo.inj_load_p + i] = (double)lp; c.inj[oo.inj_load_q + i] = (double)lq; }
        else if (!skip_inj) { inj_g[oo.inj_load_p + i] = (double)lp; inj_g[oo.inj_load_q + i] = (double)lq; }
        if (i == tid) { k9_lp0 = lp; k9_lq0 = lq; } else if (i1_) { k9_lp1 = lp; k9_lq1 = lq; }
        sum_load += (double)lp;
        if (sums_in_k9) {
          const int bu = c.load_b[i];
          if (bu >= 0) { atomicAdd(&c.Psp[bu], -(double)lp * inv_sn9); atomicAdd(&c.Qsp[bu], -(double)lq * inv_sn9); }
        }
      }
      if (lane9)
      for (int i = tid; i < g.n_gen; i += gw9)
        if (!sv.gen_slack[i]) sum_prod += (double)(i == tid ? pp_pre : ch[2 * g.n_load + i]);
      float scale_p = 1.0f;
      GPF_STAMPS(17);
      if (sa.rebalance_on) {
        G::template sum2<0>(sum_load, sum_prod);
        scale_p = (sum_prod > 0.0) ? (float)(sa.rebalance * sum_load / sum_prod) : 1.0f;
      }
      GPF_STAMPS(18);
      env_fail = false;
      float env_np = 0.f;
      if (env_on && (WPI == 1 || tid < WAVE)) {
        float np_k = tid < g.n_gen ? pp_pre : 0.f;
// ... 99 lines not shown
            any_disc = 1;
          }
        }
      }
      const bool anyd = more && G::any(any_disc);
      GPF_SYNC_IF(G::block_any_u(anyd));
      if (more && !anyd) more = false;
      if (more) tripped = true;
      if (!G::block_any_u(more)) break;
      if (more) ++rounds;
    }
    GPF_STAMPS(9);
    GPF_REDERIVE();
    if (env_on) {
      const bool ef = WPI > 1 ? (__syncthreads_or(env_fail) != 0) : env_fail;
      if (ef && st == 0) st = 6;
    }
    orow = otraj ? step * (int)b.lane_stride + inst : inst;
    if (st != 0) { write_nan_results<GW>(g, b, inst, tid, orow, otraj); a_first = __builtin_nanf(""); }
    GPF_SYNC_IF(G::block_any_u(st != 0));
    {
      const auto out = gptr(otraj ? b.traj_out : b.out) + (size_t)orow * g.n_out;
      const auto ovc = gptr(b.overflow_count) + (size_t)inst * g.n_line;
      const auto rho = gptr(b.rho) + (size_t)inst * g.n_line;
      const auto thermal_limit = gptr(b.thermal_limit);
      GPF_GLOBAL float* traj = nullptr;
      if (b.traj_rho && step < b.traj_cap) traj = gptr(b.traj_rho) + ((size_t)step * b.lane_stride + inst) * g.n_line;
      for (int l = tid; l < g.n_line; l += GW) {
        const bool own = l == tid, own2 = regs2 && l == tid + GW;
        const float lim = own ? lim_first : own2 ? lim_second : (float)thermal_limit[l];
        const float a = own ? a_first : ((st == 0 && c.out_l) ? c.out_l[oo.a_or + l] : (float)out[oo.a_or + l]);
        const float r_ = a / lim;
        if (!traj || last || sa.cascade) rho[l] = r_;
        if (traj) traj[l] = r_;
        if (!ghost) {
          const int prev = own ? ovc_first : own2 ? ovc_second : (int)ovc[l];
          const int now = (a > sa.soft_overflow * lim) ? prev + 1 : 0;
          if (own) ovc_first = now; else if (own2) ovc_second = now;
          if (!regs2 || last) ovc[l] = now;
        }
      }
      if (sa.nb_ts_reco >= 0 && st == 0 && !ghost) {
        const auto cool = gptr(b.cooldown) + (size_t)inst * g.n_line;
        const auto dround = gptr(b.disc_round) + (size_t)inst * g.n_line;
        const auto mdur = gptr(b.maint_dur) + ((size_t)tab * sa.T + row) * g.n_line;
        GPF_GLOBAL short* tcool = nullptr;
        if (b.traj_cool && step < b.traj_cap) tcool = gptr(b.traj_cool) + ((size_t)step * b.lane_stride + inst) * g.n_line;
        for (int l = tid; l < g.n_line; l += GW) {
          int cd = cool[l];
          cd = cd > 0 ? cd - 1 : 0;
          if (dround[l] >= 0) cd = sa.nb_ts_reco;
          if (b.maint_dur) { const int md = (int)mdur[l]; cd = md > cd ? md : cd; }
          cool[l] = cd;
          if (tcool) tcool[l] = (short)(cd > 32767 ? 32767 : cd);
        }
      }
    }
    const bool failed = st != 0;
    if (tid == 0) {
      const auto s = gptr(b.status) + (size_t)inst * 4;
      s[0] = st; s[1] = n_iter; s[2] = nb; s[3] = rounds;
      if (!ghost) {
        gptr(b.done)[inst] = failed ? 1 : 0;
        if (b.traj_status && step < b.traj_cap) gptr(b.traj_status)[(size_t)step * b.lane_stride + inst] = (signed char)st;
        if (failed) { if (sa.auto_reset) { ep_steps = 0; ++ep_resets; } } else ++ep_steps;
      }
    }
    if (failed && sa.auto_reset && !ghost) {
      const auto t0 = gptr(b.topo0) + (size_t)inst * g.dim_topo;
      const auto topo = gptr(b.topo) + (size_t)inst * g.dim_topo;
      const auto ovc = gptr(b.overflow_count) + (size_t)inst * g.n_line;
      for (int i = tid; i < g.dim_topo; i += GW) topo[i] = t0[i];
      for (int l = tid; l < g.n_line; l += GW) ovc[l] = 0;
      if (sa.nb_ts_reco >= 0) { const auto cool = gptr(b.cooldown) + (size_t)inst * g.n_line; for (int l = tid; l < g.n_line; l += GW) cool[l] = 0; }
      ovc_first = 0; ovc_second = 0;
      if (env_on) {
        er.target = er.actual = er.prev_p = er.amount_prev = er.curt_prev = 0.f; er.limit = 1.f; er.already = false; er.fresh = true;
        er.illegal = 0;
        er.charge = (tid < g.n_sto && P->env.charge0) ? gptr(P->env.charge0)[tid] : 0.f;
      }
    }
    reuse = !G::block_any_u(failed || tripped);
    GPF_STAMPS(7);
    if (++row >= sa.T) row = 0;
    if (!last) GPF_SYNC_IF(G::block_any_u(failed && sa.auto_reset != 0));
  }
#undef GPF_REDERIVE
#undef GPF_DCF_ON
  grp = grp0; tid = tid0; inst = inst0;
  if (keep_on) {
    const auto kb = (GPF_GLOBAL unsigned char*)sa.keep.p + (YR ? (size_t)sa.keep.stride : 0);
    const auto hdr = (GPF_GLOBAL int*)kb;
    bool won = false;
    if (keep_claim && reuse && keep_dirty && tid == 0) won = atomicCAS((int*)hdr, KEEP_KEYED, KEEP_CLAIMED) == KEEP_KEYED;
    const bool all_dcb = G::block_all_u(ts.dc_base);
    if (G::any(won)) {
      typedef double v2d_ __attribute__((ext_vector_type(2)));
      const auto km = (GPF_GLOBAL int*)(kb + sa.keep.off_m);
      const int* const img = c.btype;
      for (int i = tid; i < sa.keep.n_m; i += GW) km[i] = img[i];
      const auto ky = (GPF_GLOBAL v2d_*)(kb + sa.keep.off_y);
      auto st2 = [&](int i_, const double2 v_) { v2d_ t_; t_.x = v_.x; t_.y = v_.y; ky[i_] = t_; };
      if (YR) {
#pragma unroll
        for (int k = 0; k < YR_PASSES; ++k) {
          const int pr = tid + k * GW;
          if (pr < S.n_up) { st2(2 * pr, yreg[2 * k]); st2(2 * pr + 1, yreg[2 * k + 1]); }
        }
        if (tid < g.n_sub) st2(2 * S.n_up + tid, yreg[2 * YR_PASSES]);
      } else {
        const double2* const yl = reinterpret_cast<const double2*>(c.Yb);
        for (int i = tid; i < S.nslot_y; i += GW) st2(i, yl[i]);
      }
      const bool adc = keep_dcf && !all_dcb;
      if (adc) { const auto ka = (GPF_GLOBAL double*)(kb + sa.keep.off_d); for (int q = tid; q < S.nslot; q += GW) ka[q] = c.Adc[q]; }
      if (tid == 0) {
        hdr[1] = (ts.status & 0xff) | (ts.nb << 8);
        hdr[2] = (ts.dc_base ? 1 : 0) | (ts.gen_base ? 2 : 0) | (adc ? 4 : 0) | ((ts.dc_out + 1) << 3);
        hdr[0] = KEEP_VALID + sa.keep.launch;
      }
    }
  }
  if (tobs) {
    const int ls = sa.n_steps <= b.traj_cap ? sa.n_steps - 1 : b.traj_cap - 1;
    const size_t r = (size_t)ls * b.lane_stride + inst;
    GPF_SYNC();
    { const auto s_ = gptr(b.traj_out) + r * g.n_out; const auto d_ = gptr(b.out) + (size_t)inst * g.n_out; for (int i = tid; i < g.n_out; i += GW) d_[i] = s_[i]; }
    { const auto s_ = gptr(b.traj_topo) + r * g.dim_topo; const auto d_ = gptr(b.topo_out) + (size_t)inst * g.dim_topo; for (int i = tid; i < g.dim_topo; i += GW) d_[i] = s_[i]; }
    { const auto s_ = gptr(b.traj_shb) + r * g.n_shunt; const auto d_ = gptr(b.shunt_bus_out) + (size_t)inst * g.n_shunt; for (int i = tid; i < g.n_shunt; i += GW) d_[i] = s_[i]; }
    { const auto s_ = gptr(b.traj_lstat) + r * g.n_line; const auto d_ = gptr(b.line_status) + (size_t)inst * g.n_line; for (int i = tid; i < g.n_line; i += GW) d_[i] = s_[i]; }
  }
  if (tid == 0 && !ghost) { gptr(b.episode)[2 * (size_t)inst] = ep_steps; gptr(b.episode)[2 * (size_t)inst + 1] = ep_resets; }
  if (STAGE && !ghost) {
    const auto inj_g = gptr(b.inj) + (size_t)inst * g.n_inj;
    const int n_wb = env_on ? oo.inj_sto_q : oo.inj_sto_p;
    for (int i = tid; i < n_wb; i += GW) inj_g[i] = c.inj[i];
  }
  if (env_on && tid < LWE && !ghost) {
    const EnvDyn& E = P->env;
    if (tid < g.n_gen) {
      const size_t q = (size_t)inst * g.n_gen + tid;
      gptr(E.target)[q] = er.target; gptr(E.actual)[q] = er.actual; gptr(E.prev_p)[q] = er.prev_p; gptr(E.already)[q] = er.already ? 1 : 0;
      gptr(E.limit)[q] = er.limit;
    }
    if (tid < g.n_sto) gptr(E.charge)[(size_t)inst * g.n_sto + tid] = er.charge;
    if (tid == 0) {
      gptr(E.amount_prev)[inst] = er.amount_prev; gptr(E.curt_prev)[inst] = er.curt_prev; gptr(E.fresh)[inst] = er.fresh ? 1 : 0;
      gptr(E.illegal)[inst] = er.illegal;
    }
  }
  GPF_STAMPS(15);
  GPF_STAMPS_FLUSH(inst);
}

}
```

grid2op_amd/csrc/gridpf_symbolic.hpp:

```cpp
#pragma once
#include <algorithm>
#include <cstdint>
#include <set>
#include <vector>

namespace gpf {

struct Symbolic {
  int n = 0;
  int nslot = 0;
  int nslot_y = 0;
  int n_levels = 0;
  std::vector<int> slot_row, slot_col;
  std::vector<int> br_slot;
  std::vector<int> prog;
  int scale_off = 0, n_scale = 0;
  int back_first = -1;
  int back_off = 0;
  int max_level_piv = 0;
  int rslot0 = 0;
  int nslot_lu = 0;
  int gj_lv0 = 0;
  std::vector<int> gj_off;
  std::vector<int> gj_c, gj_r;
  std::vector<int> gj_roff;
  std::vector<int> level_of;
};

struct FlatProg {
  int gw = 0;
  bool wave_closed = true;
  unsigned solo_fwd = 0, solo_back = 0;
  int n_fwd = 0, n_scale = 0, n_scale_rhs = 0, n_back = 0;
  int scale_off = 0, back_off = 0;
  int rhs_field0 = 0;
  std::vector<int> words;
};

struct FlatProg;
inline FlatProg build_flat(const Symbolic& S, int gw, int lane_opt = 0);
inline int flat_pass_count(const Symbolic& S, int gw);
inline Symbolic build_symbolic(int n_sub, int n_line, const int* line_or_sub, const int* line_ex_sub, int degree_slack = 1, int gj_budget = -1,
                               int resched = -1) {
  if (resched < 0) {
    const int gw_nat = n_sub <= 8 ? 16 : n_sub <= 24 ? 32 : n_sub < 64 ? 64 : 128;
    Symbolic A = build_symbolic(n_sub, n_line, line_or_sub, line_ex_sub, degree_slack, gj_budget, 0);
    Symbolic B = build_symbolic(n_sub, n_line, line_or_sub, line_ex_sub, degree_slack, gj_budget, 1);
    return flat_pass_count(B, gw_nat) < flat_pass_count(A, gw_nat) ? B : A;
  }
  Symbolic S;
  S.n = n_sub;
  std::vector<std::set<int>> adj(n_sub);
  for (int l = 0; l < n_line; ++l) {
    const int a = line_or_sub[l], b = line_ex_sub[l];
    if (a != b) { adj[a].insert(b); adj[b].insert(a); }
  }
  std::vector<std::vector<std::pair<int, int>>> row_slots(n_sub);
  auto add_slot = [&](int r, int c) -> int {
    for (auto& pr : row_slots[r]) if (pr.first == c) return pr.second;
    const int s = (int)S.slot_row.size();
    S.slot_row.push_back(r);
    S.slot_col.push_back(c);
    row_slots[r].push_back({c, s});
    return s;
  };
  for (int s = 0; s < n_sub; ++s) add_slot(s, s);
  for (int s = 0; s < n_sub; ++s)
    for (int t : adj[s]) add_slot(s, t);
  S.nslot_y = (int)S.slot_row.size();
  S.br_slot.resize((size_t)4 * n_line);
  for (int l = 0; l < n_line; ++l) {
    const int a = line_or_sub[l], b = line_ex_sub[l];
    S.br_slot[4 * l + 0] = add_slot(a, a);
    S.br_slot[4 * l + 1] = add_slot(a, b);
    S.br_slot[4 * l + 2] = add_slot(b, a);
    S.br_slot[4 * l + 3] = add_slot(b, b);
  }
  struct Level {
    std::vector<int> piv, b_items, c_items, r_items;
    std::vector<std::vector<int>> u_entries;
  };
  std::vector<Level> levels;
  std::vector<std::set<int>> g = adj;
  std::vector<char> done(n_sub, 0);
  std::vector<int> asap(n_sub, 0);
  int remaining = n_sub;
  while (remaining > 0) {
    size_t mind = (size_t)-1;
    for (int s = 0; s < n_sub; ++s) if (!done[s]) mind = std::min(mind, g[s].size());
    std::vector<int> cand;
    for (int s = 0; s < n_sub; ++s) if (!done[s] && g[s].size() <= mind + (size_t)degree_slack) cand.push_back(s);
    std::stable_sort(cand.begin(), cand.end(), [&](int a, int b) { return g[a].size() < g[b].size(); });
    std::vector<char> blocked(n_sub, 0);
    Level L;
    for (int s : cand) {
      if (blocked[s]) continue;
      L.piv.push_back(s);
      blocked[s] = 1;
      for (int t : g[s]) blocked[t] = 1;
    }
    for (int p : L.piv) {
      std::vector<int> nb(g[p].begin(), g[p].end());
      std::vector<int> ue;
      for (int j : nb) {
        const int us = add_slot(p, j);
        L.b_items.push_back((p << 16) | us);
        ue.push_back((us << 16) | j);
        const int ls = add_slot(j, p);
        L.r_items.push_back(ls | (j << 16));
        L.r_items.push_back(p);
      }
      L.u_entries.push_back(ue);
      for (int i : nb)
        for (int j : nb) {
          const int dst = add_slot(i, j), ls = add_slot(i, p), us = add_slot(p, j);
          L.c_items.push_back(dst | (ls << 16));
          L.c_items.push_back(us | (p << 16));
        }
// ... 179 lines not shown
    P[S.back_off + 2 * lv + 1] = n_ent;
    if (n_ent > 0) S.back_first = lv;
  }
  return S;
}

inline std::vector<int> build_upairs(const Symbolic& S) {
  std::vector<int> up;
  for (int s = S.n; s < S.nslot_y; ++s) {
    const int r = S.slot_row[s], c = S.slot_col[s];
    if (r >= c) continue;
    int back = -1;
    for (int t = S.n; t < S.nslot_y; ++t) if (S.slot_row[t] == c && S.slot_col[t] == r) { back = t; break; }
    if (back < 0) continue;
    up.push_back(r | (c << 16));
    up.push_back(s | (back << 16));
  }
  return up;
}

inline bool flat_fits(const Symbolic& S) { return (size_t)(S.rslot0 + S.n) * 16 <= 65536; }

struct FlatAcc { unsigned rd[3]; int n_rd; unsigned at[2]; int n_at; unsigned r8; bool has_r8; bool valid; };
inline int flat_b128_group(int lane) { const int l = lane & 31; return ((l < 4 || (l >= 12 && l < 16) || (l >= 20 && l < 28)) ? 0 : 1) + 2 * ((lane >> 5) & 1); }
inline int flat_pass_cost(const std::vector<FlatAcc>& it, int gw) {
  int cost = 0;
  unsigned seen[16][8];
  int cnt[16];
  for (int base = 0; base < gw; base += 64) {
    for (int f = 0; f < 3; ++f)
      for (int g = 0; g < 4; ++g) {
        for (int q = 0; q < 16; ++q) cnt[q] = 0;
        int mx = 0;
        for (int l = 0; l < 64 && base + l < gw; ++l) {
          const FlatAcc& a = it[base + l];
          if (!a.valid || f >= a.n_rd || flat_b128_group(l) != g) continue;
          const unsigned ad = a.rd[f];
          const int q = (ad / 16) % 16;
          bool dup = false;
          for (int k = 0; k < cnt[q] && k < 8; ++k) dup |= seen[q][k] == ad;
          if (!dup) { if (cnt[q] < 8) seen[q][cnt[q]] = ad; ++cnt[q]; mx = std::max(mx, cnt[q]); }
        }
        cost += 2 * mx;
      }
    for (int g = 0; g < 4; ++g) {
      for (int f = 0; f < 3; ++f) {
        for (int q = 0; q < 16; ++q) cnt[q] = 0;
        int mx = 0;
        for (int l = 16 * g; l < 16 * g + 16 && base + l < gw; ++l) {
          const FlatAcc& a = it[base + l];
          if (!a.valid) continue;
          unsigned ad;
          if (f < 2) { if (f >= a.n_at) continue; ad = a.at[f]; }
          else { if (!a.has_r8) continue; ad = a.r8; }
          const int q = (ad / 8) % 16;
          if (f < 2) { ++cnt[q]; mx = std::max(mx, cnt[q]); }
          else {
            bool dup = false;
            for (int k = 0; k < cnt[q] && k < 8; ++k) dup |= seen[q][k] == ad;
            if (!dup) { if (cnt[q] < 8) seen[q][cnt[q]] = ad; ++cnt[q]; mx = std::max(mx, cnt[q]); }
          }
        }
        cost += 2 * mx;
      }
    }
  }
  return cost;
}
inline void flat_assign_lanes(std::vector<FlatAcc>& it, std::vector<std::pair<unsigned, unsigned>>& words, int gw, int perm_unit, int iters) {
  int cost = flat_pass_cost(it, gw);
  unsigned long long rng = 0x9E3779B97F4A7C15ull;
  auto next = [&]() { rng ^= rng << 13; rng ^= rng >> 7; rng ^= rng << 17; return (unsigned)(rng >> 32); };
  for (int k = 0; k < iters && cost > 0; ++k) {
    const int x = (int)(next() % (unsigned)gw);
    const int y = (x / perm_unit) * perm_unit + (int)(next() % (unsigned)perm_unit);
    if (x == y || (!it[x].valid && !it[y].valid)) continue;
    std::swap(it[x], it[y]);
    const int c1 = flat_pass_cost(it, gw);
    if (c1 <= cost) { cost = c1; std::swap(words[x], words[y]); }
    else std::swap(it[x], it[y]);
  }
}

inline FlatProg build_flat(const Symbolic& S, int gw, int lane_opt) {
  FlatProg F;
  F.gw = gw;
  F.rhs_field0 = S.rslot0 * 16;
  const unsigned INV = 0xffffffffu;
  auto fld = [](int slot) -> unsigned { return (unsigned)slot * 16u; };
  auto rfld = [&](int row) -> unsigned { return (unsigned)(S.rslot0 + row) * 16u; };
  std::vector<int>& W = F.words;
  const unsigned rhs0 = (unsigned)F.rhs_field0;
  auto emit_items = [&](std::vector<std::pair<unsigned, std::pair<unsigned, unsigned>>>& items, bool back) -> int {
    if (items.empty()) return 0;
    std::vector<std::pair<unsigned, unsigned>> seq;
    auto put = [&](unsigned a, unsigned b) { seq.push_back({a, b}); };
    if (gw > 64) {
      std::stable_sort(items.begin(), items.end(), [](const auto& x, const auto& y) { return x.first < y.first; });
      for (size_t i = 0; i < items.size();) {
        size_t j = i;
        while (j < items.size() && items[j].first == items[i].first) ++j;
        const size_t g = j - i, in_half = seq.size() % 64;
        const bool first_half = (seq.size() / 64) % 2 == 0 || gw != 128;
        if (g > 64) F.wave_closed = false;
        else if (in_half + g > 64 && first_half) while (seq.size() % 64) put(INV, INV);
        for (; i < j; ++i) put(items[i].second.first, items[i].second.second);
      }
    } else {
      const size_t n_pass = (items.size() + gw - 1) / gw, per = (items.size() + n_pass - 1) / n_pass;
      size_t i = 0;
      for (size_t pz = 0; pz < n_pass; ++pz) {
        for (size_t k = 0; k < per && i < items.size(); ++k, ++i) put(items[i].second.first, items[i].second.second);
        while (seq.size() % gw) put(INV, INV);
      }
    }
    while (seq.size() % gw) put(INV, INV);
    const int n_pass = (int)(seq.size() / gw);
    if (lane_opt > 0)
      for (int pz = 0; pz < n_pass; ++pz) {
        std::vector<std::pair<unsigned, unsigned>> words(seq.begin() + (size_t)pz * gw, seq.begin() + (size_t)(pz + 1) * gw);
        std::vector<FlatAcc> acc(gw);
        for (int t = 0; t < gw; ++t) {
          FlatAcc& a = acc[t];
          const unsigned w0 = words[t].first, w1 = words[t].second;
          a = FlatAcc{};
          a.valid = w0 != INV;
          if (!a.valid) continue;
          if (!back) {
            a.rd[0] = w1 >> 16; a.rd[1] = w0 >> 16; a.rd[2] = w1 & 0xffffu; a.n_rd = 3;
            a.at[0] = w0 & 0xffffu; a.at[1] = (w0 & 0xffffu) + 8; a.n_at = 2;
          } else {
            a.rd[0] = w0 & 0xffffu; a.rd[1] = (w0 >> 16) - rhs0; a.n_rd = 2;
            a.r8 = w0 >> 16; a.has_r8 = true;
            a.at[0] = w1; a.n_at = 1;
          }
        }
        flat_assign_lanes(acc, words, gw, gw > 64 ? 64 : gw, lane_opt);
        std::copy(words.begin(), words.end(), seq.begin() + (size_t)pz * gw);
      }
    if (gw > 64)
      for (int pz = 0; pz < n_pass; ++pz) {
        bool solo = true;
        for (int t = 64; t < gw; ++t) solo &= seq[(size_t)pz * gw + t].first == INV;
        const int k = (back ? F.n_back : F.n_fwd) + pz;
        if (solo && k < 32) (back ? F.solo_back : F.solo_fwd) |= 1u << k;
      }
    for (auto& w : seq) { W.push_back((int)w.first); W.push_back((int)w.second); }
    return n_pass;
  };
  for (int lv = 0; lv < S.n_levels; ++lv) {
    const int* h = S.prog.data() + (size_t)8 * lv;
    const int c_off = h[4], n_c = h[5], r_off = h[6], n_r = h[7];
    const int g0 = S.gj_off.empty() ? 0 : S.gj_off[lv], g1 = S.gj_off.empty() ? 0 : S.gj_off[lv + 1];
    const int q0 = S.gj_roff.empty() ? 0 : S.gj_roff[lv], q1 = S.gj_roff.empty() ? 0 : S.gj_roff[lv + 1];
    if (n_c + n_r + (g1 - g0) + (q1 - q0) == 0) continue;
    std::vector<std::pair<unsigned, std::pair<unsigned, unsigned>>> items;
    for (int o = g0; o < g1; o += 2) {
      const unsigned w0 = (unsigned)S.gj_c[o], w1 = (unsigned)S.gj_c[o + 1];
      items.push_back({fld(w0 & 0xffffu), {fld(w0 & 0xffffu) | (fld(w0 >> 16) << 16), fld(w1 & 0xffffu) | (fld(w1 >> 16) << 16)}});
    }
    for (int o = q0; o < q1; o += 2) {
      const unsigned w0 = (unsigned)S.gj_r[o];
      const int p = S.gj_r[o + 1];
      items.push_back({rfld((int)(w0 >> 16)), {rfld((int)(w0 >> 16)) | (fld(w0 & 0xffffu) << 16), rfld(p) | (fld(p) << 16)}});
    }
    for (int o = 0; o < n_c; ++o) {
      const unsigned w0 = (unsigned)S.prog[c_off + 2 * o], w1 = (unsigned)S.prog[c_off + 2 * o + 1];
      items.push_back({fld(w0 & 0xffffu), {fld(w0 & 0xffffu) | (fld(w0 >> 16) << 16), fld(w1 & 0xffffu) | (fld(w1 >> 16) << 16)}});
    }
    for (int o = 0; o < n_r; ++o) {
      const unsigned w0 = (unsigned)S.prog[r_off + 2 * o];
      const int p = S.prog[r_off + 2 * o + 1];
      items.push_back({rfld((int)(w0 >> 16)), {rfld((int)(w0 >> 16)) | (fld(w0 & 0xffffu) << 16), rfld(p) | (fld(p) << 16)}});
    }
    F.n_fwd += emit_items(items, false);
  }
  for (int k = 0; k < gw; ++k) { W.push_back((int)INV); W.push_back((int)INV); }
  F.scale_off = (int)W.size();
  F.n_scale = 0;
  F.n_scale_rhs = 0;
  if (W.size() & 1) W.push_back((int)INV);
  F.back_off = (int)W.size();
  for (int lv = S.back_first; lv >= 0; --lv) {
    const int ent_off = S.prog[S.back_off + 2 * lv], n_ent = S.prog[S.back_off + 2 * lv + 1];
    if (n_ent == 0 || lv >= S.gj_lv0) continue;
    std::vector<std::pair<unsigned, std::pair<unsigned, unsigned>>> items;
    for (int o = 0; o < n_ent; ++o) {
      const unsigned w = (unsigned)S.prog[ent_off + 2 * o];
      const int p = S.prog[ent_off + 2 * o + 1];
      items.push_back({rfld(p), {fld(w & 0xffffu) | (rfld((int)(w >> 16)) << 16), rfld(p)}});
    }
    F.n_back += emit_items(items, true);
  }
  for (int k = 0; k < ((gw > 64 || gw <= 32) ? 2 : 1) * gw; ++k) { W.push_back((int)INV); W.push_back((int)INV); }
  while (W.size() & 3) W.push_back((int)INV);
  return F;
}

inline int flat_pass_count(const Symbolic& S, int gw) { const FlatProg F = build_flat(S, gw, 0); return F.n_fwd + F.n_back; }

inline Symbolic relabel_slots(const Symbolic& S0, const std::vector<int>& perm) {
  Symbolic S = S0;
  for (int q = 0; q < S0.nslot; ++q) { S.slot_row[perm[q]] = S0.slot_row[q]; S.slot_col[perm[q]] = S0.slot_col[q]; }
  for (auto& v : S.br_slot) v = perm[v];
  auto lo16 = [&](int w) { return (int)(((unsigned)w & 0xffff0000u) | (unsigned)perm[(unsigned)w & 0xffffu]); };
  auto hi16 = [&](int w) { return (int)(((unsigned)w & 0xffffu) | ((unsigned)perm[(unsigned)w >> 16] << 16)); };
  for (int lv = 0; lv < S.n_levels; ++lv) {
    int* h = S.prog.data() + (size_t)8 * lv;
    for (int k = 0; k < h[3]; ++k) S.prog[h[2] + k] = lo16(S.prog[h[2] + k]);
    for (int k = 0; k < h[5]; ++k) { int& w0 = S.prog[h[4] + 2 * k]; int& w1 = S.prog[h[4] + 2 * k + 1]; w0 = hi16(lo16(w0)); w1 = lo16(w1); }
    for (int k = 0; k < h[7]; ++k) { int& w0 = S.prog[h[6] + 2 * k]; w0 = lo16(w0); }
  }
  for (int k = 0; k < S.n_scale; ++k) S.prog[S.scale_off + k] = lo16(S.prog[S.scale_off + k]);
  for (int lv = 0; lv < S.n_levels; ++lv) {
    const int off = S.prog[S.back_off + 2 * lv], n_ent = S.prog[S.back_off + 2 * lv + 1];
    for (int k = 0; k < n_ent; ++k) S.prog[off + 2 * k] = lo16(S.prog[off + 2 * k]);
  }
  for (size_t k = 0; k + 1 < S.gj_c.size(); k += 2) { S.gj_c[k] = hi16(lo16(S.gj_c[k])); S.gj_c[k + 1] = lo16(S.gj_c[k + 1]); }
  for (size_t k = 0; k + 1 < S.gj_r.size(); k += 2) S.gj_r[k] = lo16(S.gj_r[k]);
  return S;
}
inline long flat_layout_cost(const Symbolic& S, int gw) {
  const FlatProg F = build_flat(S, gw, 0);
  const unsigned INV = 0xffffffffu, rhs0 = (unsigned)F.rhs_field0;
  long tot = 0;
  std::vector<FlatAcc> acc(gw);
  auto pass = [&](int off, int k, bool back) {
    for (int t = 0; t < gw; ++t) {
      FlatAcc& a = acc[t];
      a = FlatAcc{};
      const unsigned w0 = (unsigned)F.words[off + 2 * (k * gw + t)], w1 = (unsigned)F.words[off + 2 * (k * gw + t) + 1];
      a.valid = w0 != INV;
      if (!a.valid) continue;
      if (!back) { a.rd[0] = w1 >> 16; a.rd[1] = w0 >> 16; a.rd[2] = w1 & 0xffffu; a.n_rd = 3; a.at[0] = w0 & 0xffffu; a.at[1] = (w0 & 0xffffu) + 8; a.n_at = 2; }
      else { a.rd[0] = w0 & 0xffffu; a.rd[1] = (w0 >> 16) - rhs0; a.n_rd = 2; a.r8 = w0 >> 16; a.has_r8 = true; a.at[0] = w1; a.n_at = 1; }
    }
    tot += flat_pass_cost(acc, gw);
  };
  for (int k = 0; k < F.n_fwd; ++k) pass(0, k, false);
  for (int k = 0; k < F.n_back; ++k) pass(F.back_off, k, true);
  const std::vector<int> up = build_upairs(S);
  const int n_up = (int)up.size() / 2;
  for (int k0 = 0; k0 < n_up; k0 += gw) {
    for (int t = 0; t < gw; ++t) {
      FlatAcc& a = acc[t];
      a = FlatAcc{};
      a.valid = k0 + t < n_up;
      if (!a.valid) continue;
      const unsigned w1 = (unsigned)up[2 * (k0 + t) + 1];
      a.rd[0] = (w1 & 0xffffu) * 16u; a.rd[1] = (w1 >> 16) * 16u; a.n_rd = 2;
    }
    tot += flat_pass_cost(acc, gw);
  }
  return tot;
}
inline Symbolic optimize_slot_layout(const Symbolic& S0, int iters) {
  if (iters <= 0 || S0.nslot - S0.n < 2 || !flat_fits(S0)) return S0;
  const int gw = S0.n <= 8 ? 16 : S0.n <= 24 ? 32 : S0.n < 64 ? 64 : 128;
  Symbolic cur = S0;
  long cost = flat_layout_cost(cur, gw);
// ... 20 lines not shown
```

Before: 217.0 million env steps/sec.

## Fuse first flat-LU forward pass into Newton Jacobian/mismatch assembly

When the host analysis shows that the first forward-elimination pass of the flat LU program has no read-after-write conflicts, each thread builds both its own bus block and the pivot bus block in registers. It then computes the level-0 Schur update directly and applies it with atomicAdd, so the LU starts at pass 1 and skips one synchronised pass per Newton iteration. In exchange, pivot blocks are recomputed redundantly and atomics are introduced, and the cached AOT headers are regenerated with a new fuse0 mask. Timing stamps are also added at mid-run.

Result: no change. 217.4 million env steps/sec, median of 6 (+0.2%).

```diff
diff --git a/grid2op_amd/aot/0296e7f33067.h b/grid2op_amd/aot/0296e7f33067.h
--- /dev/null
+++ b/grid2op_amd/aot/0296e7f33067.h
@@ -0,0 +1,4 @@
+#define GPF_JIT_SET_G(v) do { (v).n_sub = 118; (v).n_busbar = 2; (v).nb_tot = 236; (v).n_line = 186; (v).n_gen = 62; (v).n_load = 99; (v).n_sto = 7; (v).n_shunt = 14; (v).dim_topo = 540; (v).n_inj = 364; (v).n_out = 2574; (v).n_chron = 322; (v).sn_mva = 0x1p+0; (v).inv_sn_mva = 0x1p+0; } while (0)
+#define GPF_JIT_SET_OO(v) do { (v).p_or = 0; (v).q_or = 186; (v).v_or = 372; (v).a_or = 558; (v).th_or = 744; (v).p_ex = 930; (v).q_ex = 1116; (v).v_ex = 1302; (v).a_ex = 1488; (v).th_ex = 1674; (v).gen_p = 1860; (v).gen_q = 1922; (v).gen_v = 1984; (v).gen_th = 2046; (v).load_p = 2108; (v).load_q = 2207; (v).load_v = 2306; (v).load_th = 2405; (v).sto_p = 2504; (v).sto_q = 2511; (v).sto_v = 2518; (v).sto_th = 2525; (v).sh_p = 2532; (v).sh_q = 2546; (v).sh_v = 2560; (v).inj_gen_p = 0; (v).inj_gen_vm = 62; (v).inj_load_p = 124; (v).inj_load_q = 223; (v).inj_sto_p = 322; (v).inj_sto_q = 329; (v).inj_sh_p = 336; (v).inj_sh_q = 350; } while (0)
+#define GPF_JIT_SET_SYM(v) do { (v).n = 118; (v).nslot = 674; (v).nslot_y = 476; (v).n_levels = 13; (v).back_off = 2628; (v).n_prog = 3188; (v).scale_off = 2361; (v).n_scale = 267; (v).nslot_lu = 652; (v).n_up = 179; (v).rslot0 = 674; (v).back_first = 11; (v).static_connected = 1; (v).fuse0 = 15; (v).fl[0].n_fwd = 74; (v).fl[0].n_scale = 0; (v).fl[0].n_scale_rhs = 0; (v).fl[0].n_back = 17; (v).fl[0].scale_off = 2400; (v).fl[0].back_off = 2400; (v).fl[0].rhs_field0 = 10784; (v).fl[0].n_words = 3008; (v).fl[0].wave_closed = 1; (v).fl[0].solo_fwd = 0; (v).fl[0].solo_back = 0; (v).fl[1].n_fwd = 39; (v).fl[1].n_scale = 0; (v).fl[1].n_scale_rhs = 0; (v).fl[1].n_back = 11; (v).fl[1].scale_off = 2560; (v).fl[1].back_off = 2560; (v).fl[1].rhs_field0 = 10784; (v).fl[1].n_words = 3392; (v).fl[1].wave_closed = 1; (v).fl[1].solo_fwd = 0; (v).fl[1].solo_back = 0; (v).fl[2].n_fwd = 22; (v).fl[2].n_scale = 0; (v).fl[2].n_scale_rhs = 0; (v).fl[2].n_back = 6; (v).fl[2].scale_off = 2944; (v).fl[2].back_off = 2944; (v).fl[2].rhs_field0 = 10784; (v).fl[2].n_words = 3840; (v).fl[2].wave_closed = 1; (v).fl[2].solo_fwd = 0; (v).fl[2].solo_back = 0; (v).fl[3].n_fwd = 13; (v).fl[3].n_scale = 0; (v).fl[3].n_scale_rhs = 0; (v).fl[3].n_back = 6; (v).fl[3].scale_off = 3584; (v).fl[3].back_off = 3584; (v).fl[3].rhs_field0 = 10784; (v).fl[3].n_words = 5632; (v).fl[3].wave_closed = 1; (v).fl[3].solo_fwd = 7680; (v).fl[3].solo_back = 63; } while (0)
+#define GPF_JIT_SET_SO(v) do { (v).n_dbl = 2982; (v).n_int = 6548; (v).n_int_hot = 4024; (v).br_y = 0; (v).br_bdc = 1488; (v).sub_vn_kv = 1674; (v).shunt_fact = 1792; (v).gen_min_q = 1806; (v).gen_max_q = 1868; (v).line_vn = 1930; (v).load_vn = 2674; (v).gen_vn = 2774; (v).sto_vn = 2836; (v).shunt_vn = 2844; (v).line_ka = 2302; (v).gen_qmin_tot = 2858; (v).gen_qmax_tot = 2920; (v).gen_cnt = 5944; (v).dc_inv = -1; (v).line_or_pos = 4024; (v).line_ex_pos = 4212; (v).line_or_sub = 4400; (v).line_ex_sub = 4588; (v).br_slot = 4776; (v).gen_pos = 5520; (v).gen_sub = 5584; (v).gen_slack = 5648; (v).load_pos = 5712; (v).load_sub = 5812; (v).sto_pos = 5912; (v).sto_sub = 5920; (v).shunt_sub = 5928; (v).pair_rc = 3188; (v).up = 3664; (v).prog = 0; (v).pos_line = 6008; } while (0)
diff --git a/grid2op_amd/aot/12f4308fbc0d.h b/grid2op_amd/aot/12f4308fbc0d.h
--- /dev/null
+++ b/grid2op_amd/aot/12f4308fbc0d.h
@@ -0,0 +1,4 @@
+#define GPF_JIT_SET_G(v) do { (v).n_sub = 36; (v).n_busbar = 2; (v).nb_tot = 72; (v).n_line = 59; (v).n_gen = 22; (v).n_load = 37; (v).n_sto = 0; (v).n_shunt = 6; (v).dim_topo = 177; (v).n_inj = 130; (v).n_out = 844; (v).n_chron = 118; (v).sn_mva = 0x1p+0; (v).inv_sn_mva = 0x1p+0; } while (0)
+#define GPF_JIT_SET_OO(v) do { (v).p_or = 0; (v).q_or = 59; (v).v_or = 118; (v).a_or = 177; (v).th_or = 236; (v).p_ex = 295; (v).q_ex = 354; (v).v_ex = 413; (v).a_ex = 472; (v).th_ex = 531; (v).gen_p = 590; (v).gen_q = 612; (v).gen_v = 634; (v).gen_th = 656; (v).load_p = 678; (v).load_q = 715; (v).load_v = 752; (v).load_th = 789; (v).sto_p = 826; (v).sto_q = 826; (v).sto_v = 826; (v).sto_th = 826; (v).sh_p = 826; (v).sh_q = 832; (v).sh_v = 838; (v).inj_gen_p = 0; (v).inj_gen_vm = 22; (v).inj_load_p = 44; (v).inj_load_q = 81; (v).inj_sto_p = 118; (v).inj_sto_q = 118; (v).inj_sh_p = 118; (v).inj_sh_q = 124; } while (0)
+#define GPF_JIT_SET_SYM(v) do { (v).n = 36; (v).nslot = 196; (v).nslot_y = 146; (v).n_levels = 8; (v).back_off = 752; (v).n_prog = 920; (v).scale_off = 676; (v).n_scale = 76; (v).nslot_lu = 188; (v).n_up = 55; (v).rslot0 = 196; (v).back_first = 6; (v).static_connected = 1; (v).fuse0 = 15; (v).fl[0].n_fwd = 23; (v).fl[0].n_scale = 0; (v).fl[0].n_scale_rhs = 0; (v).fl[0].n_back = 6; (v).fl[0].scale_off = 768; (v).fl[0].back_off = 768; (v).fl[0].rhs_field0 = 3136; (v).fl[0].n_words = 1024; (v).fl[0].wave_closed = 1; (v).fl[0].solo_fwd = 0; (v).fl[0].solo_back = 0; (v).fl[1].n_fwd = 13; (v).fl[1].n_scale = 0; (v).fl[1].n_scale_rhs = 0; (v).fl[1].n_back = 3; (v).fl[1].scale_off = 896; (v).fl[1].back_off = 896; (v).fl[1].rhs_field0 = 3136; (v).fl[1].n_words = 1216; (v).fl[1].wave_closed = 1; (v).fl[1].solo_fwd = 0; (v).fl[1].solo_back = 0; (v).fl[2].n_fwd = 8; (v).fl[2].n_scale = 0; (v).fl[2].n_scale_rhs = 0; (v).fl[2].n_back = 3; (v).fl[2].scale_off = 1152; (v).fl[2].back_off = 1152; (v).fl[2].rhs_field0 = 3136; (v).fl[2].n_words = 1664; (v).fl[2].wave_closed = 1; (v).fl[2].solo_fwd = 0; (v).fl[2].solo_back = 0; (v).fl[3].n_fwd = 8; (v).fl[3].n_scale = 0; (v).fl[3].n_scale_rhs = 0; (v).fl[3].n_back = 3; (v).fl[3].scale_off = 2304; (v).fl[3].back_off = 2304; (v).fl[3].rhs_field0 = 3136; (v).fl[3].n_words = 3584; (v).fl[3].wave_closed = 1; (v).fl[3].solo_fwd = 255; (v).fl[3].solo_back = 7; } while (0)
+#define GPF_JIT_SET_SO(v) do { (v).n_dbl = 964; (v).n_int = 2020; (v).n_int_hot = 1180; (v).br_y = 0; (v).br_bdc = 472; (v).sub_vn_kv = 532; (v).shunt_fact = 568; (v).gen_min_q = 574; (v).gen_max_q = 596; (v).line_vn = 618; (v).load_vn = 854; (v).gen_vn = 892; (v).sto_vn = 914; (v).shunt_vn = 914; (v).line_ka = 736; (v).gen_qmin_tot = 920; (v).gen_qmax_tot = 942; (v).gen_cnt = 1816; (v).dc_inv = -2; (v).line_or_pos = 1180; (v).line_ex_pos = 1240; (v).line_or_sub = 1300; (v).line_ex_sub = 1360; (v).br_slot = 1420; (v).gen_pos = 1656; (v).gen_sub = 1680; (v).gen_slack = 1704; (v).load_pos = 1728; (v).load_sub = 1768; (v).sto_pos = 1808; (v).sto_sub = 1808; (v).shunt_sub = 1808; (v).pair_rc = 920; (v).up = 1068; (v).prog = 0; (v).pos_line = 1840; } while (0)
diff --git a/grid2op_amd/aot/606e1dfae8b4.h b/grid2op_amd/aot/606e1dfae8b4.h
--- /dev/null
+++ b/grid2op_amd/aot/606e1dfae8b4.h
@@ -0,0 +1,4 @@
+#define GPF_JIT_SET_G(v) do { (v).n_sub = 118; (v).n_busbar = 2; (v).nb_tot = 236; (v).n_line = 186; (v).n_gen = 62; (v).n_load = 91; (v).n_sto = 7; (v).n_shunt = 14; (v).dim_topo = 532; (v).n_inj = 348; (v).n_out = 2542; (v).n_chron = 306; (v).sn_mva = 0x1p+0; (v).inv_sn_mva = 0x1p+0; } while (0)
+#define GPF_JIT_SET_OO(v) do { (v).p_or = 0; (v).q_or = 186; (v).v_or = 372; (v).a_or = 558; (v).th_or = 744; (v).p_ex = 930; (v).q_ex = 1116; (v).v_ex = 1302; (v).a_ex = 1488; (v).th_ex = 1674; (v).gen_p = 1860; (v).gen_q = 1922; (v).gen_v = 1984; (v).gen_th = 2046; (v).load_p = 2108; (v).load_q = 2199; (v).load_v = 2290; (v).load_th = 2381; (v).sto_p = 2472; (v).sto_q = 2479; (v).sto_v = 2486; (v).sto_th = 2493; (v).sh_p = 2500; (v).sh_q = 2514; (v).sh_v = 2528; (v).inj_gen_p = 0; (v).inj_gen_vm = 62; (v).inj_load_p = 124; (v).inj_load_q = 215; (v).inj_sto_p = 306; (v).inj_sto_q = 313; (v).inj_sh_p = 320; (v).inj_sh_q = 334; } while (0)
+#define GPF_JIT_SET_SYM(v) do { (v).n = 118; (v).nslot = 674; (v).nslot_y = 476; (v).n_levels = 13; (v).back_off = 2628; (v).n_prog = 3188; (v).scale_off = 2361; (v).n_scale = 267; (v).nslot_lu = 652; (v).n_up = 179; (v).rslot0 = 674; (v).back_first = 11; (v).static_connected = 1; (v).fuse0 = 15; (v).fl[0].n_fwd = 74; (v).fl[0].n_scale = 0; (v).fl[0].n_scale_rhs = 0; (v).fl[0].n_back = 17; (v).fl[0].scale_off = 2400; (v).fl[0].back_off = 2400; (v).fl[0].rhs_field0 = 10784; (v).fl[0].n_words = 3008; (v).fl[0].wave_closed = 1; (v).fl[0].solo_fwd = 0; (v).fl[0].solo_back = 0; (v).fl[1].n_fwd = 39; (v).fl[1].n_scale = 0; (v).fl[1].n_scale_rhs = 0; (v).fl[1].n_back = 11; (v).fl[1].scale_off = 2560; (v).fl[1].back_off = 2560; (v).fl[1].rhs_field0 = 10784; (v).fl[1].n_words = 3392; (v).fl[1].wave_closed = 1; (v).fl[1].solo_fwd = 0; (v).fl[1].solo_back = 0; (v).fl[2].n_fwd = 22; (v).fl[2].n_scale = 0; (v).fl[2].n_scale_rhs = 0; (v).fl[2].n_back = 6; (v).fl[2].scale_off = 2944; (v).fl[2].back_off = 2944; (v).fl[2].rhs_field0 = 10784; (v).fl[2].n_words = 3840; (v).fl[2].wave_closed = 1; (v).fl[2].solo_fwd = 0; (v).fl[2].solo_back = 0; (v).fl[3].n_fwd = 13; (v).fl[3].n_scale = 0; (v).fl[3].n_scale_rhs = 0; (v).fl[3].n_back = 6; (v).fl[3].scale_off = 3584; (v).fl[3].back_off = 3584; (v).fl[3].rhs_field0 = 10784; (v).fl[3].n_words = 5632; (v).fl[3].wave_closed = 1; (v).fl[3].solo_fwd = 7680; (v).fl[3].solo_back = 63; } while (0)
+#define GPF_JIT_SET_SO(v) do { (v).n_dbl = 2974; (v).n_int = 6524; (v).n_int_hot = 4024; (v).br_y = 0; (v).br_bdc = 1488; (v).sub_vn_kv = 1674; (v).shunt_fact = 1792; (v).gen_min_q = 1806; (v).gen_max_q = 1868; (v).line_vn = 1930; (v).load_vn = 2674; (v).gen_vn = 2766; (v).sto_vn = 2828; (v).shunt_vn = 2836; (v).line_ka = 2302; (v).gen_qmin_tot = 2850; (v).gen_qmax_tot = 2912; (v).gen_cnt = 5928; (v).dc_inv = -1; (v).line_or_pos = 4024; (v).line_ex_pos = 4212; (v).line_or_sub = 4400; (v).line_ex_sub = 4588; (v).br_slot = 4776; (v).gen_pos = 5520; (v).gen_sub = 5584; (v).gen_slack = 5648; (v).load_pos = 5712; (v).load_sub = 5804; (v).sto_pos = 5896; (v).sto_sub = 5904; (v).shunt_sub = 5912; (v).pair_rc = 3188; (v).up = 3664; (v).prog = 0; (v).pos_line = 5992; } while (0)
diff --git a/grid2op_amd/aot/85d4f0b0125d.h b/grid2op_amd/aot/85d4f0b0125d.h
--- a/grid2op_amd/aot/85d4f0b0125d.h
+++ /dev/null
@@ -1,4 +0,0 @@
-#define GPF_JIT_SET_G(v) do { (v).n_sub = 118; (v).n_busbar = 2; (v).nb_tot = 236; (v).n_line = 186; (v).n_gen = 62; (v).n_load = 99; (v).n_sto = 7; (v).n_shunt = 14; (v).dim_topo = 540; (v).n_inj = 364; (v).n_out = 2574; (v).n_chron = 322; (v).sn_mva = 0x1p+0; (v).inv_sn_mva = 0x1p+0; } while (0)
-#define GPF_JIT_SET_OO(v) do { (v).p_or = 0; (v).q_or = 186; (v).v_or = 372; (v).a_or = 558; (v).th_or = 744; (v).p_ex = 930; (v).q_ex = 1116; (v).v_ex = 1302; (v).a_ex = 1488; (v).th_ex = 1674; (v).gen_p = 1860; (v).gen_q = 1922; (v).gen_v = 1984; (v).gen_th = 2046; (v).load_p = 2108; (v).load_q = 2207; (v).load_v = 2306; (v).load_th = 2405; (v).sto_p = 2504; (v).sto_q = 2511; (v).sto_v = 2518; (v).sto_th = 2525; (v).sh_p = 2532; (v).sh_q = 2546; (v).sh_v = 2560; (v).inj_gen_p = 0; (v).inj_gen_vm = 62; (v).inj_load_p = 124; (v).inj_load_q = 223; (v).inj_sto_p = 322; (v).inj_sto_q = 329; (v).inj_sh_p = 336; (v).inj_sh_q = 350; } while (0)
-#define GPF_JIT_SET_SYM(v) do { (v).n = 118; (v).nslot = 674; (v).nslot_y = 476; (v).n_levels = 13; (v).back_off = 2628; (v).n_prog = 3188; (v).scale_off = 2361; (v).n_scale = 267; (v).nslot_lu = 652; (v).n_up = 179; (v).rslot0 = 674; (v).back_first = 11; (v).static_connected = 1; (v).fl[0].n_fwd = 74; (v).fl[0].n_scale = 0; (v).fl[0].n_scale_rhs = 0; (v).fl[0].n_back = 17; (v).fl[0].scale_off = 2400; (v).fl[0].back_off = 2400; (v).fl[0].rhs_field0 = 10784; (v).fl[0].n_words = 3008; (v).fl[0].wave_closed = 1; (v).fl[0].solo_fwd = 0; (v).fl[0].solo_back = 0; (v).fl[1].n_fwd = 39; (v).fl[1].n_scale = 0; (v).fl[1].n_scale_rhs = 0; (v).fl[1].n_back = 11; (v).fl[1].scale_off = 2560; (v).fl[1].back_off = 2560; (v).fl[1].rhs_field0 = 10784; (v).fl[1].n_words = 3392; (v).fl[1].wave_closed = 1; (v).fl[1].solo_fwd = 0; (v).fl[1].solo_back = 0; (v).fl[2].n_fwd = 22; (v).fl[2].n_scale = 0; (v).fl[2].n_scale_rhs = 0; (v).fl[2].n_back = 6; (v).fl[2].scale_off = 2944; (v).fl[2].back_off = 2944; (v).fl[2].rhs_field0 = 10784; (v).fl[2].n_words = 3840; (v).fl[2].wave_closed = 1; (v).fl[2].solo_fwd = 0; (v).fl[2].solo_back = 0; (v).fl[3].n_fwd = 13; (v).fl[3].n_scale = 0; (v).fl[3].n_scale_rhs = 0; (v).fl[3].n_back = 6; (v).fl[3].scale_off = 3584; (v).fl[3].back_off = 3584; (v).fl[3].rhs_field0 = 10784; (v).fl[3].n_words = 5632; (v).fl[3].wave_closed = 1; (v).fl[3].solo_fwd = 7680; (v).fl[3].solo_back = 63; } while (0)
-#define GPF_JIT_SET_SO(v) do { (v).n_dbl = 2982; (v).n_int = 6548; (v).n_int_hot = 4024; (v).br_y = 0; (v).br_bdc = 1488; (v).sub_vn_kv = 1674; (v).shunt_fact = 1792; (v).gen_min_q = 1806; (v).gen_max_q = 1868; (v).line_vn = 1930; (v).load_vn = 2674; (v).gen_vn = 2774; (v).sto_vn = 2836; (v).shunt_vn = 2844; (v).line_ka = 2302; (v).gen_qmin_tot = 2858; (v).gen_qmax_tot = 2920; (v).gen_cnt = 5944; (v).dc_inv = -1; (v).line_or_pos = 4024; (v).line_ex_pos = 4212; (v).line_or_sub = 4400; (v).line_ex_sub = 4588; (v).br_slot = 4776; (v).gen_pos = 5520; (v).gen_sub = 5584; (v).gen_slack = 5648; (v).load_pos = 5712; (v).load_sub = 5812; (v).sto_pos = 5912; (v).sto_sub = 5920; (v).shunt_sub = 5928; (v).pair_rc = 3188; (v).up = 3664; (v).prog = 0; (v).pos_line = 6008; } while (0)
diff --git a/grid2op_amd/aot/c7e3abcd557d.h b/grid2op_amd/aot/c7e3abcd557d.h
--- a/grid2op_amd/aot/c7e3abcd557d.h
+++ /dev/null
@@ -1,4 +0,0 @@
-#define GPF_JIT_SET_G(v) do { (v).n_sub = 36; (v).n_busbar = 2; (v).nb_tot = 72; (v).n_line = 59; (v).n_gen = 22; (v).n_load = 37; (v).n_sto = 0; (v).n_shunt = 6; (v).dim_topo = 177; (v).n_inj = 130; (v).n_out = 844; (v).n_chron = 118; (v).sn_mva = 0x1p+0; (v).inv_sn_mva = 0x1p+0; } while (0)
-#define GPF_JIT_SET_OO(v) do { (v).p_or = 0; (v).q_or = 59; (v).v_or = 118; (v).a_or = 177; (v).th_or = 236; (v).p_ex = 295; (v).q_ex = 354; (v).v_ex = 413; (v).a_ex = 472; (v).th_ex = 531; (v).gen_p = 590; (v).gen_q = 612; (v).gen_v = 634; (v).gen_th = 656; (v).load_p = 678; (v).load_q = 715; (v).load_v = 752; (v).load_th = 789; (v).sto_p = 826; (v).sto_q = 826; (v).sto_v = 826; (v).sto_th = 826; (v).sh_p = 826; (v).sh_q = 832; (v).sh_v = 838; (v).inj_gen_p = 0; (v).inj_gen_vm = 22; (v).inj_load_p = 44; (v).inj_load_q = 81; (v).inj_sto_p = 118; (v).inj_sto_q = 118; (v).inj_sh_p = 118; (v).inj_sh_q = 124; } while (0)
-#define GPF_JIT_SET_SYM(v) do { (v).n = 36; (v).nslot = 196; (v).nslot_y = 146; (v).n_levels = 8; (v).back_off = 752; (v).n_prog = 920; (v).scale_off = 676; (v).n_scale = 76; (v).nslot_lu = 188; (v).n_up = 55; (v).rslot0 = 196; (v).back_first = 6; (v).static_connected = 1; (v).fl[0].n_fwd = 23; (v).fl[0].n_scale = 0; (v).fl[0].n_scale_rhs = 0; (v).fl[0].n_back = 6; (v).fl[0].scale_off = 768; (v).fl[0].back_off = 768; (v).fl[0].rhs_field0 = 3136; (v).fl[0].n_words = 1024; (v).fl[0].wave_closed = 1; (v).fl[0].solo_fwd = 0; (v).fl[0].solo_back = 0; (v).fl[1].n_fwd = 13; (v).fl[1].n_scale = 0; (v).fl[1].n_scale_rhs = 0; (v).fl[1].n_back = 3; (v).fl[1].scale_off = 896; (v).fl[1].back_off = 896; (v).fl[1].rhs_field0 = 3136; (v).fl[1].n_words = 1216; (v).fl[1].wave_closed = 1; (v).fl[1].solo_fwd = 0; (v).fl[1].solo_back = 0; (v).fl[2].n_fwd = 8; (v).fl[2].n_scale = 0; (v).fl[2].n_scale_rhs = 0; (v).fl[2].n_back = 3; (v).fl[2].scale_off = 1152; (v).fl[2].back_off = 1152; (v).fl[2].rhs_field0 = 3136; (v).fl[2].n_words = 1664; (v).fl[2].wave_closed = 1; (v).fl[2].solo_fwd = 0; (v).fl[2].solo_back = 0; (v).fl[3].n_fwd = 8; (v).fl[3].n_scale = 0; (v).fl[3].n_scale_rhs = 0; (v).fl[3].n_back = 3; (v).fl[3].scale_off = 2304; (v).fl[3].back_off = 2304; (v).fl[3].rhs_field0 = 3136; (v).fl[3].n_words = 3584; (v).fl[3].wave_closed = 1; (v).fl[3].solo_fwd = 255; (v).fl[3].solo_back = 7; } while (0)
-#define GPF_JIT_SET_SO(v) do { (v).n_dbl = 964; (v).n_int = 2020; (v).n_int_hot = 1180; (v).br_y = 0; (v).br_bdc = 472; (v).sub_vn_kv = 532; (v).shunt_fact = 568; (v).gen_min_q = 574; (v).gen_max_q = 596; (v).line_vn = 618; (v).load_vn = 854; (v).gen_vn = 892; (v).sto_vn = 914; (v).shunt_vn = 914; (v).line_ka = 736; (v).gen_qmin_tot = 920; (v).gen_qmax_tot = 942; (v).gen_cnt = 1816; (v).dc_inv = -2; (v).line_or_pos = 1180; (v).line_ex_pos = 1240; (v).line_or_sub = 1300; (v).line_ex_sub = 1360; (v).br_slot = 1420; (v).gen_pos = 1656; (v).gen_sub = 1680; (v).gen_slack = 1704; (v).load_pos = 1728; (v).load_sub = 1768; (v).sto_pos = 1808; (v).sto_sub = 1808; (v).shunt_sub = 1808; (v).pair_rc = 920; (v).up = 1068; (v).prog = 0; (v).pos_line = 1840; } while (0)
diff --git a/grid2op_amd/aot/c88de75e4884.h b/grid2op_amd/aot/c88de75e4884.h
--- /dev/null
+++ b/grid2op_amd/aot/c88de75e4884.h
@@ -0,0 +1,4 @@
+#define GPF_JIT_SET_G(v) do { (v).n_sub = 14; (v).n_busbar = 2; (v).nb_tot = 28; (v).n_line = 20; (v).n_gen = 6; (v).n_load = 11; (v).n_sto = 0; (v).n_shunt = 1; (v).dim_topo = 57; (v).n_inj = 36; (v).n_out = 271; (v).n_chron = 34; (v).sn_mva = 0x1.9p+6; (v).inv_sn_mva = 0x1.47ae147ae147bp-7; } while (0)
+#define GPF_JIT_SET_OO(v) do { (v).p_or = 0; (v).q_or = 20; (v).v_or = 40; (v).a_or = 60; (v).th_or = 80; (v).p_ex = 100; (v).q_ex = 120; (v).v_ex = 140; (v).a_ex = 160; (v).th_ex = 180; (v).gen_p = 200; (v).gen_q = 206; (v).gen_v = 212; (v).gen_th = 218; (v).load_p = 224; (v).load_q = 235; (v).load_v = 246; (v).load_th = 257; (v).sto_p = 268; (v).sto_q = 268; (v).sto_v = 268; (v).sto_th = 268; (v).sh_p = 268; (v).sh_q = 269; (v).sh_v = 270; (v).inj_gen_p = 0; (v).inj_gen_vm = 6; (v).inj_load_p = 12; (v).inj_load_q = 23; (v).inj_sto_p = 34; (v).inj_sto_q = 34; (v).inj_sh_p = 34; (v).inj_sh_q = 35; } while (0)
+#define GPF_JIT_SET_SYM(v) do { (v).n = 14; (v).nslot = 66; (v).nslot_y = 54; (v).n_levels = 5; (v).back_off = 242; (v).n_prog = 300; (v).scale_off = 218; (v).n_scale = 24; (v).nslot_lu = 62; (v).n_up = 20; (v).rslot0 = 66; (v).back_first = 3; (v).static_connected = 1; (v).fuse0 = 15; (v).fl[0].n_fwd = 8; (v).fl[0].n_scale = 0; (v).fl[0].n_scale_rhs = 0; (v).fl[0].n_back = 1; (v).fl[0].scale_off = 288; (v).fl[0].back_off = 288; (v).fl[0].rhs_field0 = 1056; (v).fl[0].n_words = 384; (v).fl[0].wave_closed = 1; (v).fl[0].solo_fwd = 0; (v).fl[0].solo_back = 0; (v).fl[1].n_fwd = 5; (v).fl[1].n_scale = 0; (v).fl[1].n_scale_rhs = 0; (v).fl[1].n_back = 1; (v).fl[1].scale_off = 384; (v).fl[1].back_off = 384; (v).fl[1].rhs_field0 = 1056; (v).fl[1].n_words = 576; (v).fl[1].wave_closed = 1; (v).fl[1].solo_fwd = 0; (v).fl[1].solo_back = 0; (v).fl[2].n_fwd = 5; (v).fl[2].n_scale = 0; (v).fl[2].n_scale_rhs = 0; (v).fl[2].n_back = 1; (v).fl[2].scale_off = 768; (v).fl[2].back_off = 768; (v).fl[2].rhs_field0 = 1056; (v).fl[2].n_words = 1024; (v).fl[2].wave_closed = 1; (v).fl[2].solo_fwd = 0; (v).fl[2].solo_back = 0; (v).fl[3].n_fwd = 5; (v).fl[3].n_scale = 0; (v).fl[3].n_scale_rhs = 0; (v).fl[3].n_back = 1; (v).fl[3].scale_off = 1536; (v).fl[3].back_off = 1536; (v).fl[3].rhs_field0 = 1056; (v).fl[3].n_words = 2304; (v).fl[3].wave_closed = 1; (v).fl[3].solo_fwd = 31; (v).fl[3].solo_back = 1; } while (0)
+#define GPF_JIT_SET_SO(v) do { (v).n_dbl = 516; (v).n_int = 676; (v).n_int_hot = 396; (v).br_y = 0; (v).br_bdc = 160; (v).sub_vn_kv = 180; (v).shunt_fact = 194; (v).gen_min_q = 196; (v).gen_max_q = 202; (v).line_vn = 208; (v).load_vn = 288; (v).gen_vn = 300; (v).sto_vn = 306; (v).shunt_vn = 306; (v).line_ka = 248; (v).gen_qmin_tot = 308; (v).gen_qmax_tot = 314; (v).gen_cnt = 608; (v).dc_inv = 320; (v).line_or_pos = 396; (v).line_ex_pos = 416; (v).line_or_sub = 436; (v).line_ex_sub = 456; (v).br_slot = 476; (v).gen_pos = 556; (v).gen_sub = 564; (v).gen_slack = 572; (v).load_pos = 580; (v).load_sub = 592; (v).sto_pos = 604; (v).sto_sub = 604; (v).shunt_sub = 604; (v).pair_rc = 300; (v).up = 356; (v).prog = 0; (v).pos_line = 616; } while (0)
diff --git a/grid2op_amd/aot/f41e44a3ff50.h b/grid2op_amd/aot/f41e44a3ff50.h
--- a/grid2op_amd/aot/f41e44a3ff50.h
+++ /dev/null
@@ -1,4 +0,0 @@
-#define GPF_JIT_SET_G(v) do { (v).n_sub = 118; (v).n_busbar = 2; (v).nb_tot = 236; (v).n_line = 186; (v).n_gen = 62; (v).n_load = 91; (v).n_sto = 7; (v).n_shunt = 14; (v).dim_topo = 532; (v).n_inj = 348; (v).n_out = 2542; (v).n_chron = 306; (v).sn_mva = 0x1p+0; (v).inv_sn_mva = 0x1p+0; } while (0)
-#define GPF_JIT_SET_OO(v) do { (v).p_or = 0; (v).q_or = 186; (v).v_or = 372; (v).a_or = 558; (v).th_or = 744; (v).p_ex = 930; (v).q_ex = 1116; (v).v_ex = 1302; (v).a_ex = 1488; (v).th_ex = 1674; (v).gen_p = 1860; (v).gen_q = 1922; (v).gen_v = 1984; (v).gen_th = 2046; (v).load_p = 2108; (v).load_q = 2199; (v).load_v = 2290; (v).load_th = 2381; (v).sto_p = 2472; (v).sto_q = 2479; (v).sto_v = 2486; (v).sto_th = 2493; (v).sh_p = 2500; (v).sh_q = 2514; (v).sh_v = 2528; (v).inj_gen_p = 0; (v).inj_gen_vm = 62; (v).inj_load_p = 124; (v).inj_load_q = 215; (v).inj_sto_p = 306; (v).inj_sto_q = 313; (v).inj_sh_p = 320; (v).inj_sh_q = 334; } while (0)
-#define GPF_JIT_SET_SYM(v) do { (v).n = 118; (v).nslot = 674; (v).nslot_y = 476; (v).n_levels = 13; (v).back_off = 2628; (v).n_prog = 3188; (v).scale_off = 2361; (v).n_scale = 267; (v).nslot_lu = 652; (v).n_up = 179; (v).rslot0 = 674; (v).back_first = 11; (v).static_connected = 1; (v).fl[0].n_fwd = 74; (v).fl[0].n_scale = 0; (v).fl[0].n_scale_rhs = 0; (v).fl[0].n_back = 17; (v).fl[0].scale_off = 2400; (v).fl[0].back_off = 2400; (v).fl[0].rhs_field0 = 10784; (v).fl[0].n_words = 3008; (v).fl[0].wave_closed = 1; (v).fl[0].solo_fwd = 0; (v).fl[0].solo_back = 0; (v).fl[1].n_fwd = 39; (v).fl[1].n_scale = 0; (v).fl[1].n_scale_rhs = 0; (v).fl[1].n_back = 11; (v).fl[1].scale_off = 2560; (v).fl[1].back_off = 2560; (v).fl[1].rhs_field0 = 10784; (v).fl[1].n_words = 3392; (v).fl[1].wave_closed = 1; (v).fl[1].solo_fwd = 0; (v).fl[1].solo_back = 0; (v).fl[2].n_fwd = 22; (v).fl[2].n_scale = 0; (v).fl[2].n_scale_rhs = 0; (v).fl[2].n_back = 6; (v).fl[2].scale_off = 2944; (v).fl[2].back_off = 2944; (v).fl[2].rhs_field0 = 10784; (v).fl[2].n_words = 3840; (v).fl[2].wave_closed = 1; (v).fl[2].solo_fwd = 0; (v).fl[2].solo_back = 0; (v).fl[3].n_fwd = 13; (v).fl[3].n_scale = 0; (v).fl[3].n_scale_rhs = 0; (v).fl[3].n_back = 6; (v).fl[3].scale_off = 3584; (v).fl[3].back_off = 3584; (v).fl[3].rhs_field0 = 10784; (v).fl[3].n_words = 5632; (v).fl[3].wave_closed = 1; (v).fl[3].solo_fwd = 7680; (v).fl[3].solo_back = 63; } while (0)
-#define GPF_JIT_SET_SO(v) do { (v).n_dbl = 2974; (v).n_int = 6524; (v).n_int_hot = 4024; (v).br_y = 0; (v).br_bdc = 1488; (v).sub_vn_kv = 1674; (v).shunt_fact = 1792; (v).gen_min_q = 1806; (v).gen_max_q = 1868; (v).line_vn = 1930; (v).load_vn = 2674; (v).gen_vn = 2766; (v).sto_vn = 2828; (v).shunt_vn = 2836; (v).line_ka = 2302; (v).gen_qmin_tot = 2850; (v).gen_qmax_tot = 2912; (v).gen_cnt = 5928; (v).dc_inv = -1; (v).line_or_pos = 4024; (v).line_ex_pos = 4212; (v).line_or_sub = 4400; (v).line_ex_sub = 4588; (v).br_slot = 4776; (v).gen_pos = 5520; (v).gen_sub = 5584; (v).gen_slack = 5648; (v).load_pos = 5712; (v).load_sub = 5804; (v).sto_pos = 5896; (v).sto_sub = 5904; (v).shunt_sub = 5912; (v).pair_rc = 3188; (v).up = 3664; (v).prog = 0; (v).pos_line = 5992; } while (0)
diff --git a/grid2op_amd/aot/f5e9fdf573e3.h b/grid2op_amd/aot/f5e9fdf573e3.h
--- a/grid2op_amd/aot/f5e9fdf573e3.h
+++ /dev/null
@@ -1,4 +0,0 @@
-#define GPF_JIT_SET_G(v) do { (v).n_sub = 14; (v).n_busbar = 2; (v).nb_tot = 28; (v).n_line = 20; (v).n_gen = 6; (v).n_load = 11; (v).n_sto = 0; (v).n_shunt = 1; (v).dim_topo = 57; (v).n_inj = 36; (v).n_out = 271; (v).n_chron = 34; (v).sn_mva = 0x1.9p+6; (v).inv_sn_mva = 0x1.47ae147ae147bp-7; } while (0)
-#define GPF_JIT_SET_OO(v) do { (v).p_or = 0; (v).q_or = 20; (v).v_or = 40; (v).a_or = 60; (v).th_or = 80; (v).p_ex = 100; (v).q_ex = 120; (v).v_ex = 140; (v).a_ex = 160; (v).th_ex = 180; (v).gen_p = 200; (v).gen_q = 206; (v).gen_v = 212; (v).gen_th = 218; (v).load_p = 224; (v).load_q = 235; (v).load_v = 246; (v).load_th = 257; (v).sto_p = 268; (v).sto_q = 268; (v).sto_v = 268; (v).sto_th = 268; (v).sh_p = 268; (v).sh_q = 269; (v).sh_v = 270; (v).inj_gen_p = 0; (v).inj_gen_vm = 6; (v).inj_load_p = 12; (v).inj_load_q = 23; (v).inj_sto_p = 34; (v).inj_sto_q = 34; (v).inj_sh_p = 34; (v).inj_sh_q = 35; } while (0)
-#define GPF_JIT_SET_SYM(v) do { (v).n = 14; (v).nslot = 66; (v).nslot_y = 54; (v).n_levels = 5; (v).back_off = 242; (v).n_prog = 300; (v).scale_off = 218; (v).n_scale = 24; (v).nslot_lu = 62; (v).n_up = 20; (v).rslot0 = 66; (v).back_first = 3; (v).static_connected = 1; (v).fl[0].n_fwd = 8; (v).fl[0].n_scale = 0; (v).fl[0].n_scale_rhs = 0; (v).fl[0].n_back = 1; (v).fl[0].scale_off = 288; (v).fl[0].back_off = 288; (v).fl[0].rhs_field0 = 1056; (v).fl[0].n_words = 384; (v).fl[0].wave_closed = 1; (v).fl[0].solo_fwd = 0; (v).fl[0].solo_back = 0; (v).fl[1].n_fwd = 5; (v).fl[1].n_scale = 0; (v).fl[1].n_scale_rhs = 0; (v).fl[1].n_back = 1; (v).fl[1].scale_off = 384; (v).fl[1].back_off = 384; (v).fl[1].rhs_field0 = 1056; (v).fl[1].n_words = 576; (v).fl[1].wave_closed = 1; (v).fl[1].solo_fwd = 0; (v).fl[1].solo_back = 0; (v).fl[2].n_fwd = 5; (v).fl[2].n_scale = 0; (v).fl[2].n_scale_rhs = 0; (v).fl[2].n_back = 1; (v).fl[2].scale_off = 768; (v).fl[2].back_off = 768; (v).fl[2].rhs_field0 = 1056; (v).fl[2].n_words = 1024; (v).fl[2].wave_closed = 1; (v).fl[2].solo_fwd = 0; (v).fl[2].solo_back = 0; (v).fl[3].n_fwd = 5; (v).fl[3].n_scale = 0; (v).fl[3].n_scale_rhs = 0; (v).fl[3].n_back = 1; (v).fl[3].scale_off = 1536; (v).fl[3].back_off = 1536; (v).fl[3].rhs_field0 = 1056; (v).fl[3].n_words = 2304; (v).fl[3].wave_closed = 1; (v).fl[3].solo_fwd = 31; (v).fl[3].solo_back = 1; } while (0)
-#define GPF_JIT_SET_SO(v) do { (v).n_dbl = 516; (v).n_int = 676; (v).n_int_hot = 396; (v).br_y = 0; (v).br_bdc = 160; (v).sub_vn_kv = 180; (v).shunt_fact = 194; (v).gen_min_q = 196; (v).gen_max_q = 202; (v).line_vn = 208; (v).load_vn = 288; (v).gen_vn = 300; (v).sto_vn = 306; (v).shunt_vn = 306; (v).line_ka = 248; (v).gen_qmin_tot = 308; (v).gen_qmax_tot = 314; (v).gen_cnt = 608; (v).dc_inv = 320; (v).line_or_pos = 396; (v).line_ex_pos = 416; (v).line_or_sub = 436; (v).line_ex_sub = 456; (v).br_slot = 476; (v).gen_pos = 556; (v).gen_sub = 564; (v).gen_slack = 572; (v).load_pos = 580; (v).load_sub = 592; (v).sto_pos = 604; (v).sto_sub = 604; (v).shunt_sub = 604; (v).pair_rc = 300; (v).up = 356; (v).prog = 0; (v).pos_line = 616; } while (0)
diff --git a/grid2op_amd/csrc/gridpf_capi.hip b/grid2op_amd/csrc/gridpf_capi.hip
--- a/grid2op_amd/csrc/gridpf_capi.hip
+++ b/grid2op_amd/csrc/gridpf_capi.hip
@@ -196,6 +196,7 @@
 
 bool upload_flats(const gpf::Symbolic& S, DevArr<int>& buf, gpf::SymDev& D, int lane_opt = 0) {
   D.rslot0 = S.rslot0;
+  D.fuse0 = 0;
   for (int k = 0; k < 4; ++k) { D.flat[k] = nullptr; D.fl[k] = gpf::FlatDev{}; }
   if (!gpf::flat_fits(S)) return true;
   std::vector<int> all;
@@ -231,6 +232,7 @@
     f.n_fwd = F.n_fwd; f.n_scale = F.n_scale; f.n_scale_rhs = F.n_scale_rhs; f.n_back = F.n_back; f.scale_off = F.scale_off;
     f.back_off = F.back_off; f.rhs_field0 = F.rhs_field0; f.n_words = (int)F.words.size(); f.wave_closed = F.wave_closed ? 1 : 0;
     f.solo_fwd = (int)F.solo_fwd; f.solo_back = (int)F.solo_back;
+    if (F.fuse0) D.fuse0 |= 1 << k;
   }
   if (buf.upload(all.data(), all.size()) != hipSuccess) return false;
   for (int k = 0; k < 4; ++k) D.flat[k] = buf.p + off[k];
diff --git a/grid2op_amd/csrc/gridpf_sparse.hpp b/grid2op_amd/csrc/gridpf_sparse.hpp
--- a/grid2op_amd/csrc/gridpf_sparse.hpp
+++ b/grid2op_amd/csrc/gridpf_sparse.hpp
@@ -78,6 +78,7 @@
   int nslot_lu;
   int n_up;
   int rslot0;
+  int fuse0;
   const int* flat[4];
   FlatDev fl[4];
   int back_first;
@@ -90,7 +91,8 @@
 };
 
 #define GPF_SYMDEV_INTS(X) X(n) X(nslot) X(nslot_y) X(n_levels) X(back_off) X(n_prog) X(scale_off) X(n_scale) X(nslot_lu) X(n_up) X(rslot0) X(back_first) \
-  X(static_connected)
+  X(static_connected) X(fuse0)
+static_assert(offsetof(SymDev, flat) == 48 && offsetof(SymDev, fuse0) == 44, "SymDev::fuse0 sits in the alignment gap in front of SymDev::flat");
 
 struct TopoClassDev {
   SymDev sym;
@@ -113,7 +115,7 @@
 };
 
 #ifdef GPF_TIMING
-constexpr int GPF_NSTAMP = 40;
+constexpr int GPF_NSTAMP = 42;
 constexpr int GPF_NPASS_T = 48;
 constexpr int GPF_WORK_ROW = GPF_NSTAMP + GPF_NPASS_T;
 static __shared__ long long gpf_pass_t[GPF_NPASS_T];
@@ -613,9 +615,9 @@
   }
 }
 
-template <int GW, class PP = const int*, bool RES = false>
+template <int GW, class PP = const int*, bool RES = false, bool FUSABLE = false>
 __device__ inline bool block_lu_flat(const FlatDev& F, PP prog, double* __restrict__ A, size_t HS, int tid, long long* dbg = nullptr,
-                                     const FlatWords<RES>* W = nullptr) {
+                                     const FlatWords<RES>* W = nullptr, int fwd0 = 0) {
 #ifdef GPF_TIMING
   const long long t_lu0 = __builtin_readcyclecounter();
 #endif
@@ -634,7 +636,7 @@
 #else
 #define GPF_PASS_T(i_) do {} while (0)
 #endif
-  GPF_PASS_T(0);
+  GPF_PASS_T(FUSABLE ? fwd0 : 0);
   auto fwd_item = [&](const unsigned w0, const unsigned w1) {
     if (w0 != 0xffffffffu) {
       const unsigned fd = w0 & 0xffffu, fl = w0 >> 16, fu = w1 & 0xffffu, fp = w1 >> 16;
@@ -653,7 +655,7 @@
       }
     }
   };
-#define GPF_WALK(n_, at0_, MASK_, NEXT_SOLO_, ITEM_, TB_, WR_, CAP_)                                                                                 \
+#define GPF_WALK(n_, at0_, MASK_, NEXT_SOLO_, ITEM_, TB_, WR_, CAP_, K0_)                                                                            \
   {                                                                                                                                \
     const unsigned solo_ = GW > WAVE ? (unsigned)(MASK_) : 0u;                                                                     \
     const int n_pass_ = (n_);                                                                                                      \
@@ -668,14 +670,14 @@
     if constexpr (RES) {                                   \
       _Pragma("unroll")                                                                                                            \
       for (int k = 0; k < (CAP_); ++k)                                                                                             \
-        if (k < n_pass_) step_(W->WR_[2 * k], W->WR_[2 * k + 1], k);                                                               \
+        if (k >= (K0_) && k < n_pass_) step_(W->WR_[2 * k], W->WR_[2 * k + 1], k);                                                 \
     } else {                                                                                                                       \
-    int at = (at0_) + 2 * tid;                                                                                                     \
+    int at = (at0_) + 2 * tid + 2 * GW * (K0_);                                                                                    \
     unsigned p0 = (unsigned)prog[at], p1 = (unsigned)prog[at + 1];                                                                 \
     if (PF2) {                                                                                                                     \
       at += 2 * GW;                                                                                                                \
       unsigned q0 = (unsigned)prog[at], q1 = (unsigned)prog[at + 1], r0, r1;                                                       \
-      for (int k = 0; k < n_pass_; k += 3) {                                                                                       \
+      for (int k = (K0_); k < n_pass_; k += 3) {                                                                                   \
         at += 2 * GW; r0 = (unsigned)prog[at]; r1 = (unsigned)prog[at + 1];                                                        \
         step_(p0, p1, k);                                                                                                          \
         if (k + 1 >= n_pass_) break;                                                                                               \
@@ -686,7 +688,7 @@
         step_(r0, r1, k + 2);                                                                                                      \
       }                                                                                                                            \
     } else {                                                                                                                       \
-      for (int k = 0; k < n_pass_; ++k) {                                                                                          \
+      for (int k = (K0_); k < n_pass_; ++k) {                                                                                      \
         at += 2 * GW;                                                                                                              \
         const unsigned n0 = (unsigned)prog[at], n1 = (unsigned)prog[at + 1];                           \
         step_(p0, p1, k);                                                                                                          \
@@ -695,7 +697,8 @@
     }                                                                                                                              \
     }                                                                                                                              \
   }
-  GPF_WALK(F.n_fwd, 0, F.solo_fwd, F.n_back > 0 && (F.solo_back & 1), fwd_item, 1, f, GPF_WR_CAP_F)
+  const int k_first = FUSABLE ? fwd0 : 0;
+  GPF_WALK(F.n_fwd, 0, F.solo_fwd, F.n_back > 0 && (F.solo_back & 1), fwd_item, 1, f, GPF_WR_CAP_F, k_first)
 #ifdef GPF_TIMING
   const long long t_lu1 = __builtin_readcyclecounter();
 #endif
@@ -710,7 +713,7 @@
       atomicAdd(FL_D(a1, w1), -fma(uB.x, x0, uB.y * x1));
     }
   };
-  GPF_WALK(F.n_back, F.back_off, F.solo_back, false, back_item, 1 + F.n_fwd, b, GPF_WR_CAP_B)
+  GPF_WALK(F.n_back, F.back_off, F.solo_back, false, back_item, 1 + F.n_fwd, b, GPF_WR_CAP_B, 0)
 #ifdef GPF_TIMING
   if (dbg) { dbg[0] = t_lu1 - t_lu0; dbg[1] = (long long)__builtin_readcyclecounter() - t_lu1; }
 #endif
@@ -744,7 +747,7 @@
   };
 #undef GPF_PASS_T
 #define GPF_PASS_T(i_) do {} while (0)
-  GPF_WALK(F.n_fwd, 0, F.solo_fwd, F.n_back > 0 && (F.solo_back & 1), fwd_item, 0, f, GPF_WR_CAP_F)
+  GPF_WALK(F.n_fwd, 0, F.solo_fwd, F.n_back > 0 && (F.solo_back & 1), fwd_item, 0, f, GPF_WR_CAP_F, 0)
 #ifdef GPF_TIMING
   const long long t_lu1 = __builtin_readcyclecounter();
 #endif
@@ -754,7 +757,7 @@
       atomicAdd(FL_D(a0, w1), -(*facp(w0 & 0xffffu) * *FL_D(a0, fj)) * fast_rcp(*facp(fj - (unsigned)F.rhs_field0)));
     }
   };
-  GPF_WALK(F.n_back, F.back_off, F.solo_back, false, back_item, 0, b, GPF_WR_CAP_B)
+  GPF_WALK(F.n_back, F.back_off, F.solo_back, false, back_item, 0, b, GPF_WR_CAP_B, 0)
 #ifdef GPF_TIMING
   if (dbg) { dbg[0] = t_lu1 - t_lu0; dbg[1] = (long long)__builtin_readcyclecounter() - t_lu1; }
 #endif
@@ -764,6 +767,27 @@
 #undef GPF_WALK
 #undef FL_LD2
 #undef FL_D
+
+#ifdef GPF_FUSE_P0
+template <int NB, int IPW, int WPI> constexpr bool fuse_p0_ct() { return NB == 1 && IPW > 1 && WPI == 1; }
+#else
+template <int NB, int IPW, int WPI> constexpr bool fuse_p0_ct() { return false; }
+#endif
+__device__ __forceinline__ void nwr_bus_block(const double2 ydiag, const double e, const double f, const double ivm, double& Sr, double& Si,
+                                              const bool diag_on, const bool rowP, const bool rowQ, const double psp, const double qsp,
+                                              double2& d0, double2& d1, double& mp, double& mq) {
+#pragma clang fp contract(off)
+  const double aa = fma(ydiag.x, e, -(ydiag.y * f)), bb = fma(ydiag.x, f, ydiag.y * e);
+  const double tr_ = fma(e, aa, f * bb);
+  const double ti_ = fma(f, aa, -(e * bb));
+  if (diag_on) { Sr += tr_; Si += ti_; }
+  const double2 r0 = make_double2(rowP ? ti_ : 0.0, (rowP && rowQ) ? tr_ * ivm : 0.0);
+  const double2 r1 = make_double2((rowQ && rowP) ? -tr_ : 0.0, rowQ ? ti_ * ivm : 0.0);
+  d0 = make_double2(rowP ? r0.x - Si : 1.0, rowQ ? fma(Sr, ivm, r0.y) : r0.y);
+  d1 = make_double2(rowQ ? r1.x + Sr : r1.x, rowQ ? fma(Si, ivm, r1.y) : 1.0);
+  mp = rowP ? (Sr - psp) : 0.0;
+  mq = rowQ ? (Si - qsp) : 0.0;
+}
 
 struct SolveCtl {
   bool inj_staged;
@@ -1124,6 +1148,10 @@
     }
     if (STAGE >= 1) return block_lu_solve<BS, GW>(S, sv.prog.p, c.A, c.rhs, tid, dbg);
     return block_lu_solve<BS, GW>(S, gptr(sv.prog.p), c.A, c.rhs, tid, dbg);
+  };
+  auto lu_ac_from = [&](long long* dbg, const int fwd0) -> bool {
+    if (WRES && wres) return block_lu_flat<GW, decltype(gptr(flat_g)), WRES, true>(FL, gptr(flat_g), c.A, HS, tid, dbg, &FW, fwd0);
+    return block_lu_flat<GW, decltype(gptr(flat_g)), false, true>(FL, gptr(flat_g), c.A, HS, tid, dbg, nullptr, fwd0);
   };
   auto lu_dc = [&](long long* dbg) -> bool {
     if (dc_kept) {
@@ -1227,6 +1255,27 @@
 #define NWR_YD (KEEP_Y ? ydiag0 : *p_yd)
 #define NWR_PSP (KEEP_Y ? psp0 : c.Psp[ib])
 #define NWR_QSP (KEEP_Y ? qsp0 : c.Qsp[ib])
+      constexpr bool FUSE_CT = fuse_p0_ct<NB, IPW, WPI>();
+      const bool fuse0 = FUSE_CT && ((S.fuse0 >> gw_index(GW)) & 1) != 0;
+      unsigned fw0 = 0xffffffffu, fw1 = 0u;
+      if (fuse0) {
+        if constexpr (WRES) { if (wres) { fw0 = FW.f[0]; fw1 = FW.f[1]; } }
+        if (!(WRES && wres)) { fw0 = (unsigned)gptr(flat_g)[2 * tid]; fw1 = (unsigned)gptr(flat_g)[2 * tid + 1]; }
+      }
+      const bool it_on = fuse0 && fw0 != 0xffffffffu;
+      const unsigned f_d = it_on ? (fw0 & 0xffffu) : 0u, f_l = it_on ? (fw0 >> 16) : 0u, f_p = it_on ? (fw1 >> 16) : 0u;
+      const bool u_rhs = it_on && (fw1 & 0xffffu) >= (unsigned)FL.rhs_field0;
+      const unsigned f_u = (it_on && !u_rhs) ? (fw1 & 0xffffu) : 0u;
+      const int pv = (int)(f_p >> 4);
+      const double2* const p_ydp = reinterpret_cast<const double2*>(c.Yb + (size_t)pv * 2);
+      const double2 ydp0 = *p_ydp;
+      const int btp = c.btype[pv];
+      const double pspp0 = c.Psp[pv], qspp0 = c.Qsp[pv];
+      const bool prowP = (btp == BT_PQ || btp == BT_PV), prowQ = (btp == BT_PQ);
+      const bool pdiag_on = btp != BT_OFF && (ydp0.x != 0.0 || ydp0.y != 0.0);
+#define NWR_YDP (KEEP_Y ? ydp0 : *p_ydp)
+#define NWR_PSPP (KEEP_Y ? pspp0 : c.Psp[pv])
+#define NWR_QSPP (KEEP_Y ? qspp0 : c.Qsp[pv])
       double va, vm;
 #ifdef GPF_TIMING
       asm volatile("s_waitcnt lgkmcnt(0)" ::: "memory");
@@ -1304,6 +1353,56 @@
         if (it == 0) GPF_STAMPS(11);
         double fabs_mis = 0.0;
         bool bad = false;
+        if (FUSE_CT && fuse0) {
+          const char* const a0 = reinterpret_cast<const char*>(c.A);
+          const char* const a1 = a0 + HS * 8;
+          Sr = *SreP(ib); Si = *SimP(ib);
+          double Spr = *SreP(pv), Spi = *SimP(pv);
+          const double2 efp = EF(pv);
+          const double ivmp = c.ivm[pv];
+          const double2 lA = *reinterpret_cast<const double2*>(a0 + f_l), lB = *reinterpret_cast<const double2*>(a1 + f_l);
+          const double2 uA_l = *reinterpret_cast<const double2*>(a0 + f_u), uB_l = *reinterpret_cast<const double2*>(a1 + f_u);
+          double2 d0, d1, p0, p1;
+          double mp, mq, pmp, pmq;
+          nwr_bus_block(NWR_YD, e, f, ivm, Sr, Si, diag_on, rowP, rowQ, NWR_PSP, NWR_QSP, d0, d1, mp, mq);
+          const double am = fmax(fabs(mp), fabs(mq));
+          bad = b_on && !(am <= 1e300);
+          fabs_mis = b_on ? am : 0.0;
+          nwr_bus_block(NWR_YDP, efp.x, efp.y, ivmp, Spr, Spi, pdiag_on, prowP, prowQ, NWR_PSPP, NWR_QSPP, p0, p1, pmp, pmq);
+          const double2 dA = p0, dB = p1;
+          const double2 uA = u_rhs ? make_double2(-pmp, 0.0) : uA_l, uB = u_rhs ? make_double2(-pmq, 0.0) : uB_l;
+          const double rd = -fast_rcp(fma(dA.x, dB.y, -dA.y * dB.x));
+          const double t00 = fma(lA.x, dB.y, -lA.y * dB.x), t01 = fma(lA.y, dA.x, -lA.x * dA.y);
+          const double t10 = fma(lB.x, dB.y, -lB.y * dB.x), t11 = fma(lB.y, dA.x, -lB.x * dA.y);
+          const double x00 = fma(t00, uA.x, t01 * uB.x) * rd, x10 = fma(t10, uA.x, t11 * uB.x) * rd;
+          const double x01 = fma(t00, uA.y, t01 * uB.y) * rd, x11 = fma(t10, uA.y, t11 * uB.y) * rd;
+          if (!done) {
+            const unsigned fl = G::template any2<0>(!(fabs_mis < tol_pu), bad);
+            if (fl & 2u) { status = 1; done = true; }
+            else if (!(fl & 1u)) { converged = true; done = true; }
+            else if (it >= max_iter) done = true;
+            else ++it;
+          }
+          if (G::block_all_u(done)) break;
+          if (b_on) {
+            *reinterpret_cast<double2*>(Ad0) = d0;
+            *reinterpret_cast<double2*>(Ad1) = d1;
+            *rhsT(ib) = -mp; *rhsV(ib) = -mq;
+          }
+          asm volatile("" ::: "memory");
+          if (it_on) {
+            double* const q0 = reinterpret_cast<double*>(const_cast<char*>(a0) + f_d);
+            double* const q1 = reinterpret_cast<double*>(const_cast<char*>(a1) + f_d);
+            atomicAdd(&q0[0], x00);
+            atomicAdd(&q1[0], x10);
+            if (f_d < (unsigned)FL.rhs_field0) {
+              atomicAdd(&q0[1], x01);
+              atomicAdd(&q1[1], x11);
+            }
+          }
+          GPF_LSYNC();
+          if (it == 1) GPF_STAMPS(12);
+        } else {
         if (b_on) {
           Sr = *SreP(ib); Si = *SimP(ib);
           const double2 ydiag = NWR_YD;
@@ -1332,11 +1431,15 @@
         if (G::block_all_u(done)) break;
         GPF_LSYNC();
         if (it == 1) GPF_STAMPS(12);
+        }
 #ifdef GPF_TIMING
-        const bool ok = lu_ac(it == 1 ? &stamps.v[32] : nullptr);
+        long long* const lu_dbg = it == 1 ? &stamps.v[32] : nullptr;
 #else
-        const bool ok = lu_ac(nullptr);
-#endif
+        long long* const lu_dbg = nullptr;
+#endif
+        bool ok;
+        if constexpr (FUSE_CT) ok = lu_ac_from(lu_dbg, fuse0 ? 1 : 0);
+        else ok = lu_ac(lu_dbg);
         if (it == 1) GPF_STAMPS(13);
         bool fin = true, piv_ok = true;
         if (b_on) {
@@ -1373,6 +1476,9 @@
 #undef NWR_YD
 #undef NWR_PSP
 #undef NWR_QSP
+#undef NWR_YDP
+#undef NWR_PSPP
+#undef NWR_QSPP
     } else {
       for (int i = tid; i < nbus; i += GW) {
         const double va = c.va[i], vmi = c.vm[i];
@@ -2379,6 +2485,7 @@
     const bool otraj = tobs && step < b.traj_cap;
     int orow = otraj ? step * (int)b.lane_stride + inst : inst;
     GPF_STAMPS(19);
+    if (step == sa.n_steps / 2) GPF_STAMPS(40);
     bool sums_in_k9 = false, skip_inj = false;
     float k9_lp0 = 0.f, k9_lq0 = 0.f, k9_lp1 = 0.f, k9_lq1 = 0.f, k9_pp = 0.f, k9_vm = 1.f;
     {
@@ -2644,6 +2751,7 @@
     }
     reuse = !G::block_any_u(failed || tripped);
     GPF_STAMPS(7);
+    if (step == sa.n_steps / 2) GPF_STAMPS(41);
     if (++row >= sa.T) row = 0;
     if (!last) GPF_SYNC_IF(G::block_any_u(failed && sa.auto_reset != 0));
   }
diff --git a/grid2op_amd/csrc/gridpf_symbolic.hpp b/grid2op_amd/csrc/gridpf_symbolic.hpp
--- a/grid2op_amd/csrc/gridpf_symbolic.hpp
+++ b/grid2op_amd/csrc/gridpf_symbolic.hpp
@@ -34,6 +34,7 @@
   int n_fwd = 0, n_scale = 0, n_scale_rhs = 0, n_back = 0;
   int scale_off = 0, back_off = 0;
   int rhs_field0 = 0;
+  bool fuse0 = false;
   std::vector<int> words;
 };
 
@@ -379,6 +380,21 @@
   }
 }
 
+inline bool flat_fuse0(const std::vector<int>& words, int n_fwd, int gw, int rhs_field0) {
+  if (n_fwd < 1) return false;
+  std::vector<char> is_dst(2 * 65536 / 16, 0);
+  for (int t = 0; t < gw; ++t) {
+    const unsigned w0 = (unsigned)words[2 * t];
+    if (w0 != 0xffffffffu) is_dst[(w0 & 0xffffu) / 16] = 1;
+  }
+  for (int t = 0; t < gw; ++t) {
+    const unsigned w0 = (unsigned)words[2 * t], fp = (unsigned)words[2 * t + 1] >> 16;
+    if (w0 == 0xffffffffu) continue;
+    if (is_dst[fp / 16] || is_dst[(fp + (unsigned)rhs_field0) / 16]) return false;
+  }
+  return true;
+}
+
 inline FlatProg build_flat(const Symbolic& S, int gw, int lane_opt) {
   FlatProg F;
   F.gw = gw;
@@ -473,6 +489,7 @@
     F.n_fwd += emit_items(items, false);
   }
   for (int k = 0; k < gw; ++k) { W.push_back((int)INV); W.push_back((int)INV); }
+  F.fuse0 = flat_fuse0(W, F.n_fwd, gw, F.rhs_field0);
   F.scale_off = (int)W.size();
   F.n_scale = 0;
   F.n_scale_rhs = 0;
```
